# lzzcd001/MeshDiffusion

Measured on NVIDIA H100. Metric: denoising sample-steps/sec at res-64 (4x64^3), uncond_gen PC sampler, higher is better.
Workload: dtype bf16x3

## Files before the change

include/meshdiff_b200.h:

```cpp
#ifndef MESHDIFF_B200_H
#define MESHDIFF_B200_H

#ifdef __cplusplus
extern "C" {
#endif

const char* mdb_last_error(void);
int mdb_version(void);

typedef struct mdb_unet mdb_unet;

typedef struct mdb_unet_config {
  int image_size;
  int nf;
  int n_levels;
  int ch_mult[8];
  int num_res_blocks;
  int level0_blocks;
  int n_attn;
  int attn_resolutions[4];
  int num_channels;
  int stem_ksize;
  int use_pos_bias;
  int max_batch;
  int precision;
  int training;
} mdb_unet_config;

int mdb_unet_create(const mdb_unet_config* cfg, mdb_unet** out);
int mdb_unet_create_dry(const mdb_unet_config* cfg, mdb_unet** out);
void mdb_unet_destroy(mdb_unet* net);

int mdb_unet_num_params(mdb_unet* net);
int mdb_unet_param_info(mdb_unet* net, int idx, const char** name, long long* numel, int* ndim, long long* shape8);
int mdb_unet_set_param(mdb_unet* net, const char* name, const float* src, long long numel, int src_is_device,
                       void* stream);
int mdb_unet_set_params(mdb_unet* net, int count, const char* const* names, const float* const* srcs, const long long* numels,
                        void* stream);
int mdb_unet_get_param(mdb_unet* net, const char* name, float* dst, long long numel, int dst_is_device, void* stream);
int mdb_unet_commit(mdb_unet* net, void* stream);
int mdb_unet_forward(mdb_unet* net, const float* x, const float* labels, float* out, int batch, void* stream);
int mdb_unet_info(mdb_unet* net, double* flops_per_sample, long long* arena_bytes, int* n_gemm_launches, int* n_steps);
int mdb_unet_gemm_ops(mdb_unet* net, int i, const char** name, double* flops, double* fill_bytes);
int mdb_unet_gemm_slots(mdb_unet* net, int i, int* a_slots, int* b_slots, int* smem_bytes);
int mdb_unet_gemm_tiles(mdb_unet* net, int i, int* work_items, int* splits, int* ksteps, int* entry_ksteps, int* block_n);
int mdb_unet_profile(mdb_unet* net, const float* x, const float* labels, float* out, int batch, void* stream,
                     char* names_buf, int names_len, float* ms, int max_steps, int* n_steps);

int mdb_unet_set_dropout(mdb_unet* net, float p, unsigned long long seed);
int mdb_unet_backward(mdb_unet* net, const float* dout, float* grads, long long grads_numel, int batch, int accumulate,
                      void* stream);
int mdb_unet_grad_offset(mdb_unet* net, const char* name, long long* offset);
int mdb_unet_backward_input(mdb_unet* net, const float* dout, float* dx, float* grads, long long grads_numel, int batch,
                            int accumulate, void* stream);
int mdb_unet_grad_ready(mdb_unet* net, const char* name, int* n_launches);
int mdb_unet_backward_marked(mdb_unet* net, const float* dout, float* grads, long long grads_numel, int batch,
                             int accumulate, const int* mark_steps, void* const* mark_events, int n_marks, void* stream);
int mdb_unet_debug_stats(mdb_unet* net, long long* host_out, long long capacity, long long* count);
int mdb_unet_train_info(mdb_unet* net, double* bwd_flops_per_sample, int* n_bwd_steps, long long* total_param_numel);
int mdb_unet_profile_backward(mdb_unet* net, const float* dout, float* grads, int batch, void* stream, char* names_buf,
                              int names_len, float* ms, int max_steps, int* n_steps);

int mdb_fingerprint(const void* const* ptrs_dev, const long long* numels_dev, int n, unsigned long long* out_dev,
                    void* stream);

typedef struct mdb_sampler_cond {
  const float* partial;
  long long partial_bstride;
  const float* partial_mask;
  long long mask_bstride;
  int channel;
  float mean_coef, std;
  const float* noise;
} mdb_sampler_cond;

int mdb_sampler_update(const float* eps, float* x, float* x_mean, const float* noise, const float* mask, float beta,
                       float std, long long voxels, int channels, int batch, unsigned long long seed,
                       unsigned long long offset, const mdb_sampler_cond* cond , void* stream);
int mdb_sampler_run(mdb_unet* net, float* x, float* x_mean, const float* mask, const float* labels,
                    const float* betas, const float* stds, int n_steps, int batch, unsigned long long seed,
                    float* eps_buf, float* labels_buf, int step0, const mdb_sampler_cond* cond ,
                    const float* cond_mean_coefs, const float* cond_stds, int cond_until, void* stream);

typedef struct mdb_solver_step {
  float label;
  float sigma, inv_alpha;
  float c_x, c_0, c_1, c_z;
  float cond_coef, cond_std;
} mdb_solver_step;

int mdb_solver_update(const float* eps, float* x, float* x0_hist, const float* mask, const mdb_solver_step* step,
                      long long voxels, int channels, int batch, const float* noise ,
                      unsigned long long seed, unsigned long long offset, const mdb_sampler_cond* cond ,
                      void* stream);
int mdb_solver_run(mdb_unet* net, float* x, float* x0_hist, const float* mask, const mdb_solver_step* steps, int n_steps,
                   int batch, unsigned long long seed, float* eps_buf, float* labels_buf, int step0,
                   const mdb_sampler_cond* cond , int cond_until, void* stream);

int mdb_ddpm_loss(const float* pred, const float* noise, const float* mask, double mask_sum, float* loss_out,
                  float* grad_pred, double* scratch, int batch, int channels, long long voxels, void* stream);
int mdb_ddpm_perturb(const float* x0, const float* noise, const float* mask, const float* sqrt_ac,
                     const float* sqrt_1mac, float* out, int batch, int channels, long long voxels, void* stream);
int mdb_chunk_elems(void);
int mdb_grad_clip_coef(const float* const* grads_dev, const long long* numels_dev, const int* chunks_dev, int n_chunks,
                       float max_norm, float* coef_out, float* total_norm_out, double* scratch, void* stream);
int mdb_adam_ema_step(float* const* params_dev, const float* const* grads_dev, float* const* exp_avg_dev,
                      float* const* exp_avg_sq_dev, float* const* ema_dev, const long long* numels_dev,
                      const int* chunks_dev, int n_chunks, float lr, float beta1, float beta2, float eps,
                      float weight_decay, int step, const float* clip_coef_dev, float ema_decay, void* stream);
int mdb_ema_update(float* const* ema_dev, const float* const* params_dev, const long long* numels_dev,
                   const int* chunks_dev, int n_chunks, float ema_decay, void* stream);

int mdb_allreduce_grads(void* nccl_comm, float* grads, long long numel, int world_size, void* stream);

int mdb_conv3d(const void* x, int batch, int cin, int z, int y_, int x_, const float* w, const float* bias, int cout,
               int ksize, int stride, void* out, const float* rowbias, const void* residual, long long* stats,
               int precision, void* stream);
int mdb_groupnorm_act(const void* x, const long long* stats, const float* gamma, const float* beta, void* y, int batch,
                      long long voxels, int channels, int silu, int precision, void* stream);

int mdb_conv3d_backward(const void* dy, const void* x, const float* w, int batch, int cin, int cout, int z, int y_,
                        int x_, int ksize, int stride, float* dw, void* dx, void* stream);
int mdb_conv3d_backward_prec(const void* dy, const void* x, const float* w, int batch, int cin, int cout, int z, int y_,
                             int x_, int ksize, int stride, float* dw, void* dx, int precision, void* stream);
int mdb_groupnorm_act_backward(const void* x, const long long* stats, const float* gamma, const float* beta,
                               void* da, const void* add, void* dx, float* dgamma, float* dbeta, int batch,
                               long long voxels, int channels, int silu, float dropout_p, unsigned long long seed,
                               void* stream);
int mdb_groupnorm_act_backward_prec(const void* x, const long long* stats, const float* gamma, const float* beta,
                                    void* da, const void* add, void* dx, float* dgamma, float* dbeta, int batch,
                                    long long voxels, int channels, int silu, float dropout_p, unsigned long long seed,
                                    int precision, void* stream);

int mdb_marching_tets_prepare(const int* tets_host, int n_tets, int n_verts, int max_batch, void** handle);
void mdb_marching_tets_destroy(void* handle);
int mdb_marching_tets_info(void* handle, int* n_edges, int* uv_grid_n);
int mdb_marching_tets_uvs(void* handle, float* uvs, void* stream);
int mdb_marching_tets_count(void* handle, const float* sdf, int batch, int* counts_host, void* stream);
int mdb_marching_tets_extract(void* handle, const float* pos, long long pos_batch_stride, const float* sdf, int batch,
                              float* verts, long long* faces, long long* uv_idx, long long* face_to_tet,
                              long long* valid_vert_idx, const long long* vert_off, const long long* face_off,
                              const long long* vv_off, void* stream);
int mdb_marching_tets_vertex_ids(void* handle, int batch, unsigned* out, void* stream);
int mdb_marching_tets_backward(void* handle, const float* pos, long long pos_batch_stride, const float* sdf, int batch,
                               const unsigned* vertex_ids, const float* grad_verts, const long long* vert_off,
                               float* grad_pos, float* grad_sdf, void* stream);

int mdb_mesh_auto_normals(const float* v_pos, const long long* faces, int n_verts, int n_faces, float* v_nrm, float* f_nrm,
                          long long* scratch, void* stream);
int mdb_mesh_compute_tangents(const float* v_pos, const long long* t_pos_idx, const float* v_tex, const long long* t_tex_idx,
                              const float* v_nrm, const long long* t_nrm_idx, int n_nrm, int n_faces, float* v_tng,
                              long long* scratch, void* stream);

int mdb_mesh_sample_points(const float* verts, const long long* faces, const long long* vert_off, const long long* face_off,
                           int n_meshes, int n_points, const float* uniforms, unsigned long long seed, long long first_id,
                           double* cdf, float* points, int* n_written, void* stream);
int mdb_chamfer_matrix(const float* A, int nA, int N, const float* B, int nB, int M, double* out, void* stream);
int mdb_emd_matrix(const float* A, int nA, const float* B, int nB, int N, float eps, double* out, double* gap, void* stream);

int mdb_pflow_drift_div(const float* x, const float* e, const float* h, const float* g, const float* mask, float beta, float std,
                        float* drift, double* div, int batch, int channels, long long voxels, void* stream);

int mdb_raster_depth(const float* verts, const long long* faces, const long long* vert_off, const long long* face_off,
                     const int* job_mesh, const float* mvp, int n_jobs, int res, unsigned long long* scratch, float* depth,
                     int* face_id, int* n_behind, void* stream);
int mdb_visible_tets(const float* pos, long long pos_stride, const int* tets, int n_tets, const long long* face_to_tet,
                     const long long* face_off, const int* job_mesh, const float* mvp, int n_jobs, int res, const float* depth,
                     const int* face_id, unsigned char* visible, unsigned char* rast, void* stream);

#ifdef __cplusplus
}
#endif
#endif
```

meshdiffusion_b200/_native.py:

```python
import ctypes
import os

_HERE = os.path.dirname(os.path.abspath(__file__))
LIB_PATH = os.path.join(_HERE, "lib", "libmeshdiff_b200.so")

_lib = None


class NativeError(RuntimeError):
    pass


class UNetConfigC(ctypes.Structure):
    _fields_ = [
        ("image_size", ctypes.c_int),
        ("nf", ctypes.c_int),
        ("n_levels", ctypes.c_int),
        ("ch_mult", ctypes.c_int * 8),
        ("num_res_blocks", ctypes.c_int),
        ("level0_blocks", ctypes.c_int),
        ("n_attn", ctypes.c_int),
        ("attn_resolutions", ctypes.c_int * 4),
        ("num_channels", ctypes.c_int),
        ("stem_ksize", ctypes.c_int),
        ("use_pos_bias", ctypes.c_int),
        ("max_batch", ctypes.c_int),
        ("precision", ctypes.c_int),
        ("training", ctypes.c_int),
    ]


class SamplerCondC(ctypes.Structure):
    _fields_ = [
        ("partial", ctypes.c_void_p), ("partial_bstride", ctypes.c_longlong),
        ("partial_mask", ctypes.c_void_p), ("mask_bstride", ctypes.c_longlong),
        ("channel", ctypes.c_int), ("mean_coef", ctypes.c_float), ("std", ctypes.c_float),
        ("noise", ctypes.c_void_p),
    ]


class SolverStepC(ctypes.Structure):
    _fields_ = [(name, ctypes.c_float) for name in
                ("label", "sigma", "inv_alpha", "c_x", "c_0", "c_1", "c_z", "cond_coef", "cond_std")]


_vp, _i, _ll, _f, _u64, _d = ctypes.c_void_p, ctypes.c_int, ctypes.c_longlong, ctypes.c_float, ctypes.c_ulonglong, ctypes.c_double
SIGNATURES = {
    "mdb_last_error": (ctypes.c_char_p, []),
    "mdb_version": (_i, []),
    "mdb_unet_create": (_i, [ctypes.POINTER(UNetConfigC), ctypes.POINTER(_vp)]),
    "mdb_unet_create_dry": (_i, [ctypes.POINTER(UNetConfigC), ctypes.POINTER(_vp)]),
    "mdb_unet_destroy": (None, [_vp]),
    "mdb_unet_num_params": (_i, [_vp]),
    "mdb_unet_param_info": (_i, [_vp, _i, ctypes.POINTER(ctypes.c_char_p), ctypes.POINTER(_ll), ctypes.POINTER(_i), ctypes.POINTER(_ll)]),
    "mdb_unet_set_param": (_i, [_vp, ctypes.c_char_p, _vp, _ll, _i, _vp]),
    "mdb_unet_get_param": (_i, [_vp, ctypes.c_char_p, _vp, _ll, _i, _vp]),
    "mdb_unet_commit": (_i, [_vp, _vp]),
    "mdb_unet_set_params": (_i, [_vp, _i, _vp, _vp, _vp, _vp]),
    "mdb_unet_forward": (_i, [_vp, _vp, _vp, _vp, _i, _vp]),
    "mdb_unet_info": (_i, [_vp, ctypes.POINTER(_d), ctypes.POINTER(_ll), ctypes.POINTER(_i), ctypes.POINTER(_i)]),
    "mdb_unet_gemm_ops": (_i, [_vp, _i, ctypes.POINTER(ctypes.c_char_p), ctypes.POINTER(_d), ctypes.POINTER(_d)]),
    "mdb_unet_gemm_slots": (_i, [_vp, _i, ctypes.POINTER(_i), ctypes.POINTER(_i), ctypes.POINTER(_i)]),
    "mdb_unet_gemm_tiles": (_i, [_vp, _i, ctypes.POINTER(_i), ctypes.POINTER(_i), ctypes.POINTER(_i), ctypes.POINTER(_i),
                                 ctypes.POINTER(_i)]),
    "mdb_unet_profile": (_i, [_vp, _vp, _vp, _vp, _i, _vp, ctypes.c_char_p, _i, ctypes.POINTER(_f), _i, ctypes.POINTER(_i)]),
    "mdb_unet_set_dropout": (_i, [_vp, _f, _u64]),
    "mdb_unet_backward": (_i, [_vp, _vp, _vp, _ll, _i, _i, _vp]),
    "mdb_unet_grad_offset": (_i, [_vp, ctypes.c_char_p, ctypes.POINTER(_ll)]),
    "mdb_unet_backward_input": (_i, [_vp, _vp, _vp, _vp, _ll, _i, _i, _vp]),
    "mdb_unet_grad_ready": (_i, [_vp, ctypes.c_char_p, ctypes.POINTER(_i)]),
    "mdb_unet_backward_marked": (_i, [_vp, _vp, _vp, _ll, _i, _i, ctypes.POINTER(_i), ctypes.POINTER(_vp), _i, _vp]),
    "mdb_unet_debug_stats": (_i, [_vp, _vp, _ll, ctypes.POINTER(_ll)]),
    "mdb_unet_train_info": (_i, [_vp, ctypes.POINTER(_d), ctypes.POINTER(_i), ctypes.POINTER(_ll)]),
    "mdb_unet_profile_backward": (_i, [_vp, _vp, _vp, _i, _vp, ctypes.c_char_p, _i, ctypes.POINTER(_f), _i, ctypes.POINTER(_i)]),
    "mdb_fingerprint": (_i, [_vp, _vp, _i, _vp, _vp]),
    "mdb_sampler_update": (_i, [_vp, _vp, _vp, _vp, _vp, _f, _f, _ll, _i, _i, _u64, _u64, ctypes.POINTER(SamplerCondC), _vp]),
    "mdb_sampler_run": (_i, [_vp, _vp, _vp, _vp, ctypes.POINTER(_f), ctypes.POINTER(_f), ctypes.POINTER(_f), _i, _i, _u64, _vp, _vp,
                             _i, ctypes.POINTER(SamplerCondC), ctypes.POINTER(_f), ctypes.POINTER(_f), _i, _vp]),
    "mdb_solver_update": (_i, [_vp, _vp, _vp, _vp, ctypes.POINTER(SolverStepC), _ll, _i, _i, _vp, _u64, _u64,
                               ctypes.POINTER(SamplerCondC), _vp]),
    "mdb_solver_run": (_i, [_vp, _vp, _vp, _vp, ctypes.POINTER(SolverStepC), _i, _i, _u64, _vp, _vp, _i,
                            ctypes.POINTER(SamplerCondC), _i, _vp]),
    "mdb_ddpm_loss": (_i, [_vp, _vp, _vp, _d, _vp, _vp, _vp, _i, _i, _ll, _vp]),
    "mdb_ddpm_perturb": (_i, [_vp, _vp, _vp, _vp, _vp, _vp, _i, _i, _ll, _vp]),
    "mdb_chunk_elems": (_i, []),
    "mdb_grad_clip_coef": (_i, [_vp, _vp, _vp, _i, _f, _vp, _vp, _vp, _vp]),
    "mdb_adam_ema_step": (_i, [_vp, _vp, _vp, _vp, _vp, _vp, _vp, _i, _f, _f, _f, _f, _f, _i, _vp, _f, _vp]),
    "mdb_ema_update": (_i, [_vp, _vp, _vp, _vp, _i, _f, _vp]),
    "mdb_allreduce_grads": (_i, [_vp, _vp, _ll, _i, _vp]),
    "mdb_conv3d": (_i, [_vp, _i, _i, _i, _i, _i, _vp, _vp, _i, _i, _i, _vp, _vp, _vp, _vp, _i, _vp]),
    "mdb_groupnorm_act": (_i, [_vp, _vp, _vp, _vp, _vp, _i, _ll, _i, _i, _i, _vp]),
    "mdb_conv3d_backward": (_i, [_vp, _vp, _vp, _i, _i, _i, _i, _i, _i, _i, _i, _vp, _vp, _vp]),
    "mdb_groupnorm_act_backward": (_i, [_vp, _vp, _vp, _vp, _vp, _vp, _vp, _vp, _vp, _i, _ll, _i, _i, _f, _u64, _vp]),
    "mdb_conv3d_backward_prec": (_i, [_vp, _vp, _vp, _i, _i, _i, _i, _i, _i, _i, _i, _vp, _vp, _i, _vp]),
    "mdb_groupnorm_act_backward_prec": (_i, [_vp, _vp, _vp, _vp, _vp, _vp, _vp, _vp, _vp, _i, _ll, _i, _i, _f, _u64, _i, _vp]),
    "mdb_marching_tets_prepare": (_i, [_vp, _i, _i, _i, ctypes.POINTER(_vp)]),
    "mdb_marching_tets_destroy": (None, [_vp]),
    "mdb_marching_tets_info": (_i, [_vp, ctypes.POINTER(_i), ctypes.POINTER(_i)]),
    "mdb_marching_tets_uvs": (_i, [_vp, _vp, _vp]),
    "mdb_marching_tets_count": (_i, [_vp, _vp, _i, ctypes.POINTER(_i), _vp]),
    "mdb_mesh_auto_normals": (_i, [_vp, _vp, _i, _i, _vp, _vp, _vp, _vp]),
    "mdb_mesh_compute_tangents": (_i, [_vp, _vp, _vp, _vp, _vp, _vp, _i, _i, _vp, _vp, _vp]),
    "mdb_marching_tets_extract": (_i, [_vp, _vp, _ll, _vp, _i, _vp, _vp, _vp, _vp, _vp, _vp, _vp, _vp, _vp]),
    "mdb_marching_tets_vertex_ids": (_i, [_vp, _i, _vp, _vp]),
    "mdb_marching_tets_backward": (_i, [_vp, _vp, _ll, _vp, _i, _vp, _vp, _vp, _vp, _vp, _vp]),
    "mdb_mesh_sample_points": (_i, [_vp, _vp, _vp, _vp, _i, _i, _vp, _u64, _ll, _vp, _vp, _vp, _vp]),
    "mdb_chamfer_matrix": (_i, [_vp, _i, _i, _vp, _i, _i, _vp, _vp]),
    "mdb_emd_matrix": (_i, [_vp, _i, _vp, _i, _i, _f, _vp, _vp, _vp]),
    "mdb_pflow_drift_div": (_i, [_vp, _vp, _vp, _vp, _vp, _f, _f, _vp, _vp, _i, _i, _ll, _vp]),
    "mdb_raster_depth": (_i, [_vp, _vp, _vp, _vp, _vp, _vp, _i, _i, _vp, _vp, _vp, _vp, _vp]),
    "mdb_visible_tets": (_i, [_vp, _ll, _vp, _i, _vp, _vp, _vp, _vp, _i, _i, _vp, _vp, _vp, _vp, _vp]),
}


def lib():
    global _lib
    if _lib is not None:
        return _lib
    if not os.path.exists(LIB_PATH):
        from . import build as _build
        _build.build()
    if not os.path.exists(LIB_PATH):
        raise NativeError("libmeshdiff_b200.so is missing and could not be built; there is no fallback path")
    L = ctypes.CDLL(LIB_PATH)
    for name, (res, args) in SIGNATURES.items():
        fn = getattr(L, name)
        fn.restype = res
        fn.argtypes = args
    _lib = L
    return L


def check(code):
    if code != 0:
        raise NativeError(lib().mdb_last_error().decode())


def ptr(t):
    if t is None:
        return None
    return ctypes.c_void_p(t.data_ptr())


def current_stream():
    import torch
    return ctypes.c_void_p(torch.cuda.current_stream().cuda_stream)
```

meshdiffusion_b200/csrc/api.cu:

```cuda
#include "../../include/meshdiff_b200.h"
#include "unet.h"
#include <cstring>
#include <cmath>

using namespace mdb;

static thread_local std::string g_err;
namespace mdb { void set_last_error(const std::string& msg) { g_err = msg; } }

#define MDB_API_BEGIN try {
#define MDB_API_END                         \
  }                                         \
  catch (const std::exception& e) {         \
    g_err = e.what();                       \
    return 1;                               \
  }                                         \
  catch (...) {                             \
    g_err = "mdb: unknown error";           \
    return 2;                               \
  }                                         \
  return 0;

struct mdb_unet { UNet* net; };

extern "C" {

const char* mdb_last_error(void) { return g_err.c_str(); }
int mdb_version(void) { return 100; }

static int create_impl(const mdb_unet_config* c, mdb_unet** out, bool dry) {
  MDB_API_BEGIN
  if (!c || !out) throw std::runtime_error("mdb: null argument");
  UNetConfig u;
  u.image_size = c->image_size; u.nf = c->nf; u.n_levels = c->n_levels;
  for (int i = 0; i < 8; ++i) u.ch_mult[i] = c->ch_mult[i];
  u.num_res_blocks = c->num_res_blocks; u.level0_blocks = c->level0_blocks;
  u.n_attn = c->n_attn;
  for (int i = 0; i < 4; ++i) u.attn_resolutions[i] = c->attn_resolutions[i];
  u.num_channels = c->num_channels; u.stem_ksize = c->stem_ksize; u.use_pos_bias = c->use_pos_bias;
  u.max_batch = c->max_batch; u.precision = c->precision; u.training = c->training;
  auto* h = new mdb_unet;
  h->net = nullptr;
  try { h->net = new UNet(u, dry); } catch (...) { delete h; throw; }
  *out = h;
  MDB_API_END
}

int mdb_unet_create(const mdb_unet_config* c, mdb_unet** out) { return create_impl(c, out, false); }
int mdb_unet_create_dry(const mdb_unet_config* c, mdb_unet** out) { return create_impl(c, out, true); }

void mdb_unet_destroy(mdb_unet* n) {
  if (!n) return;
  delete n->net;
  delete n;
}

int mdb_unet_num_params(mdb_unet* n) { return n ? (int)n->net->params().size() : -1; }

int mdb_unet_param_info(mdb_unet* n, int idx, const char** name, long long* numel, int* ndim, long long* shape8) {
  MDB_API_BEGIN
  const auto& ps = n->net->params();
  if (idx < 0 || idx >= (int)ps.size()) throw std::runtime_error("mdb: parameter index out of range");
  if (name) *name = ps[idx].name.c_str();
  if (numel) *numel = ps[idx].numel;
  if (ndim) *ndim = (int)ps[idx].shape.size();
  if (shape8) for (size_t i = 0; i < ps[idx].shape.size() && i < 8; ++i) shape8[i] = ps[idx].shape[i];
  MDB_API_END
}

int mdb_unet_set_param(mdb_unet* n, const char* name, const float* src, long long numel, int dev, void* stream) {
  MDB_API_BEGIN
  n->net->set_param(name, src, numel, dev != 0, (cudaStream_t)stream);
  MDB_API_END
}

int mdb_unet_set_params(mdb_unet* n, int count, const char* const* names, const float* const* srcs, const long long* numels,
                        void* stream) {
  MDB_API_BEGIN
  for (int i = 0; i < count; ++i) n->net->set_param(names[i], srcs[i], numels[i], true, (cudaStream_t)stream);
  MDB_API_END
}

int mdb_unet_get_param(mdb_unet* n, const char* name, float* dst, long long numel, int dev, void* stream) {
  MDB_API_BEGIN
  n->net->get_param(name, dst, numel, dev != 0, (cudaStream_t)stream);
  MDB_API_END
}

int mdb_unet_commit(mdb_unet* n, void* stream) {
  MDB_API_BEGIN
  n->net->commit((cudaStream_t)stream);
  MDB_API_END
}

int mdb_unet_forward(mdb_unet* n, const float* x, const float* labels, float* out, int B, void* stream) {
  MDB_API_BEGIN
  n->net->forward(x, labels, out, B, (cudaStream_t)stream);
  MDB_API_END
}

int mdb_unet_info(mdb_unet* n, double* flops, long long* arena, int* ngemm, int* nsteps) {
  MDB_API_BEGIN
  if (flops) *flops = n->net->flops_per_sample();
  if (arena) *arena = (long long)n->net->arena_bytes();
  if (ngemm) *ngemm = n->net->num_gemm_launches();
  if (nsteps) *nsteps = n->net->num_steps();
  MDB_API_END
}

int mdb_unet_gemm_ops(mdb_unet* n, int i, const char** name, double* flops, double* fill_bytes) {
  MDB_API_BEGIN
  if (i < 0 || i >= n->net->num_gemm_launches()) throw std::runtime_error("mdb: GEMM launch index out of range");
  const GemmOp& g = n->net->gemm(i);
  if (name) *name = g.name.c_str();
  if (flops) *flops = g.flops;
  if (fill_bytes) *fill_bytes = g.fill_bytes();
  MDB_API_END
}

int mdb_unet_gemm_slots(mdb_unet* n, int i, int* a_slots, int* b_slots, int* smem_bytes) {
  MDB_API_BEGIN
  if (i < 0 || i >= n->net->num_gemm_launches()) throw std::runtime_error("mdb: GEMM launch index out of range");
  int a = 0, b = 0, sm = 0;
  n->net->gemm(i).slots(a, b, sm);
  if (a_slots) *a_slots = a;
  if (b_slots) *b_slots = b;
  if (smem_bytes) *smem_bytes = sm;
  MDB_API_END
}

int mdb_unet_gemm_tiles(mdb_unet* n, int i, int* work_items, int* splits, int* ksteps, int* entry_ksteps, int* block_n) {
  MDB_API_BEGIN
  if (i < 0 || i >= n->net->num_gemm_launches()) throw std::runtime_error("mdb: GEMM launch index out of range");
  const GemmOp& g = n->net->gemm(i);
  const int s = g.p.splits > 1 ? g.p.splits : 1;
  int nk = 0;
  for (const LoadEntry& e : g.loads) nk = e.nk > nk ? e.nk : nk;
  if (work_items) *work_items = g.p.tx * g.p.ty * g.p.tz * g.p.tb * g.p.n_tiles_n * s;
  if (splits) *splits = s;
  if (ksteps) *ksteps = g.ksteps;
  if (entry_ksteps) *entry_ksteps = nk;
  if (block_n) *block_n = g.block_n;
  MDB_API_END
}

int mdb_unet_profile(mdb_unet* n, const float* x, const float* labels, float* out, int B, void* stream, char* names,
                     int names_len, float* ms, int max_steps, int* nsteps) {
  MDB_API_BEGIN
  auto r = n->net->profile(x, labels, out, B, (cudaStream_t)stream);
  std::string all;
  int k = 0;
  for (auto& p : r) {
    if (k >= max_steps) break;
    all += p.first; all += "\n";
    ms[k++] = p.second;
  }
  if ((int)all.size() + 1 > names_len) throw std::runtime_error("mdb: names buffer too small");
  std::memcpy(names, all.c_str(), all.size() + 1);
  if (nsteps) *nsteps = k;
  MDB_API_END
}

int mdb_unet_set_dropout(mdb_unet* n, float p, unsigned long long seed) {
  MDB_API_BEGIN
  n->net->set_dropout(p, seed);
  MDB_API_END
}

int mdb_unet_backward(mdb_unet* n, const float* dout, float* grads, long long grads_numel, int B, int accumulate, void* stream) {
  MDB_API_BEGIN
  if (grads_numel != n->net->total_param_numel()) throw std::runtime_error("mdb: gradient buffer has the wrong size");
  n->net->backward(dout, grads, B, accumulate != 0, (cudaStream_t)stream);
  MDB_API_END
}

int mdb_unet_backward_marked(mdb_unet* n, const float* dout, float* grads, long long grads_numel, int B, int accumulate,
                             const int* mark_steps, void* const* mark_events, int n_marks, void* stream) {
  MDB_API_BEGIN
  if (grads_numel != n->net->total_param_numel()) throw std::runtime_error("mdb: gradient buffer has the wrong size");
  if (n_marks > 0 && (!mark_steps || !mark_events)) throw std::runtime_error("mdb: null mark arrays");
  n->net->backward(dout, grads, B, accumulate != 0, (cudaStream_t)stream, mark_steps, mark_events, n_marks);
  MDB_API_END
}

int mdb_unet_backward_input(mdb_unet* n, const float* dout, float* dx, float* grads, long long grads_numel, int B, int accumulate,
                            void* stream) {
  MDB_API_BEGIN
  if (grads && grads_numel != n->net->total_param_numel()) throw std::runtime_error("mdb: gradient buffer has the wrong size");
  n->net->backward_input(dout, dx, grads, B, accumulate != 0, (cudaStream_t)stream);
  MDB_API_END
}

int mdb_unet_grad_ready(mdb_unet* n, const char* name, int* step) {
  MDB_API_BEGIN
  *step = n->net->grad_ready_step(name);
  MDB_API_END
}

int mdb_unet_grad_offset(mdb_unet* n, const char* name, long long* off) {
  MDB_API_BEGIN
  *off = n->net->grad_offset(name);
  MDB_API_END
}

int mdb_unet_debug_stats(mdb_unet* n, long long* host_out, long long capacity, long long* count) {
  MDB_API_BEGIN
  const long long c = (long long)n->net->stats_count();
  if (count) *count = c;
  if (host_out) {
    if (capacity < c) throw std::runtime_error("mdb: stats buffer too small");
    MDB_CUDA_CHECK(cudaMemcpy(host_out, n->net->stats_ptr(), (size_t)c * sizeof(long long), cudaMemcpyDeviceToHost));
  }
  MDB_API_END
}

int mdb_unet_train_info(mdb_unet* n, double* bwd_flops, int* nsteps, long long* numel) {
  MDB_API_BEGIN
  if (bwd_flops) *bwd_flops = n->net->bwd_flops_per_sample();
  if (nsteps) *nsteps = n->net->num_bwd_steps();
  if (numel) *numel = n->net->total_param_numel();
  MDB_API_END
}

int mdb_unet_profile_backward(mdb_unet* n, const float* dout, float* grads, int B, void* stream, char* names, int names_len,
                              float* ms, int max_steps, int* nsteps) {
  MDB_API_BEGIN
  auto r = n->net->profile_backward(dout, grads, B, (cudaStream_t)stream);
  std::string all;
  int k = 0;
  for (auto& p : r) {
    if (k >= max_steps) break;
    all += p.first; all += "\n";
    ms[k++] = p.second;
  }
  if ((int)all.size() + 1 > names_len) throw std::runtime_error("mdb: names buffer too small");
  std::memcpy(names, all.c_str(), all.size() + 1);
  if (nsteps) *nsteps = k;
  MDB_API_END
}

static void set_cond(SamplerUpdateArgs& a, const mdb_sampler_cond* c, float coef, float stdv) {
  if (!c || !c->partial) return;
  if (!c->partial_mask) throw std::runtime_error("mdb: conditional sampling needs partial_mask");
  if (c->channel < 0 || c->channel >= a.C) throw std::runtime_error("mdb: partial_channel out of range");
  a.cond_partial = c->partial; a.cond_partial_bs = c->partial_bstride;
  a.cond_pmask = c->partial_mask; a.cond_pmask_bs = c->mask_bstride;
  a.cond_channel = c->channel; a.cond_coef = coef; a.cond_std = stdv; a.cond_noise = c->noise;
}

int mdb_sampler_update(const float* eps, float* x, float* x_mean, const float* noise, const float* mask, float beta,
                       float stdv, long long V, int C, int B, unsigned long long seed, unsigned long long offset,
                       const mdb_sampler_cond* cond, void* stream) {
  MDB_API_BEGIN
  SamplerUpdateArgs a{};
  a.eps = eps; a.x = x; a.x_mean = x_mean; a.noise = noise; a.mask = mask; a.beta = beta; a.stdv = stdv;
  a.V = V; a.C = C; a.seed = seed; a.offset = offset;
  if (cond) set_cond(a, cond, cond->mean_coef, cond->std);
  launch_sampler_update(a, B, (cudaStream_t)stream);
  MDB_API_END
}

__global__ void fingerprint_kernel(const unsigned int* const* ptrs, const long long* numels, unsigned long long* out) {
  const int t = blockIdx.y;
  const unsigned int* p = ptrs[t];
  const long long n = numels[t];
  unsigned long long h = 0;
  for (long long i = blockIdx.x * (long long)blockDim.x + threadIdx.x; i < n; i += (long long)gridDim.x * blockDim.x)
    h += (unsigned long long)p[i] * (0x9E3779B97F4A7C15ull * (unsigned long long)(i + 1) | 1ull);
  for (int o = 16; o; o >>= 1) h += __shfl_xor_sync(0xffffffffu, h, o);
  if ((threadIdx.x & 31) == 0 && h) atomicAdd(out + t, h);
}

int mdb_fingerprint(const void* const* ptrs_dev, const long long* numels_dev, int n, unsigned long long* out_dev, void* stream) {
  MDB_API_BEGIN
  cudaStream_t s = (cudaStream_t)stream;
  MDB_CUDA_CHECK(cudaMemsetAsync(out_dev, 0, (size_t)n * 8, s));
  fingerprint_kernel<<<dim3(64, n), 256, 0, s>>>(reinterpret_cast<const unsigned int* const*>(ptrs_dev), numels_dev, out_dev);
  MDB_CUDA_CHECK(cudaGetLastError());
  MDB_API_END
}

__global__ void fill_kernel(float* p, float v, int n) {
  const int i = blockIdx.x * blockDim.x + threadIdx.x;
  if (i < n) p[i] = v;
}

int mdb_sampler_run(mdb_unet* n, float* x, float* x_mean, const float* mask, const float* labels, const float* betas,
                    const float* stds, int n_steps, int B, unsigned long long seed, float* eps_buf, float* labels_buf,
                    int step0, const mdb_sampler_cond* cond, const float* cond_mean_coefs, const float* cond_stds,
                    int cond_until, void* stream) {
  MDB_API_BEGIN
  cudaStream_t s = (cudaStream_t)stream;
  const UNetConfig& c = n->net->cfg();
  const long long V = (long long)c.image_size * c.image_size * c.image_size;
  if (cond && cond->partial && (!cond_mean_coefs || !cond_stds)) throw std::runtime_error("mdb: conditional run needs the marginal_prob tables");
  if (cond && cond->noise) throw std::runtime_error("mdb: mdb_sampler_run draws its noise in-kernel (cond->noise must be NULL)");
  for (int i = 0; i < n_steps; ++i) {
    fill_kernel<<<(B + 127) / 128, 128, 0, s>>>(labels_buf, labels[i], B);
    n->net->forward(x, labels_buf, eps_buf, B, s, true);
    SamplerUpdateArgs a{};
    a.eps = eps_buf; a.x = x; a.x_mean = x_mean; a.noise = nullptr; a.mask = mask; a.beta = betas[i]; a.stdv = stds[i];
    a.V = V; a.C = c.num_channels; a.seed = seed; a.offset = 4ull * (unsigned long long)(step0 + i);
    if (cond && step0 + i < cond_until) set_cond(a, cond, cond_mean_coefs[i], cond_stds[i]);
    launch_sampler_update(a, B, s);
  }
  MDB_API_END
}

static SolverUpdateArgs solver_args(const float* eps, float* x, float* x0_hist, const float* mask, const mdb_solver_step& st,
                                    long long V, int C, const mdb_sampler_cond* c) {
  SolverUpdateArgs a{};
  a.eps = eps; a.x = x; a.x0_hist = x0_hist; a.mask = mask;
  a.sigma = st.sigma; a.inv_alpha = st.inv_alpha; a.c_x = st.c_x; a.c_0 = st.c_0; a.c_1 = st.c_1; a.c_z = st.c_z;
  a.V = V; a.C = C;
  if (c && c->partial) {
    if (!c->partial_mask) throw std::runtime_error("mdb: conditional sampling needs partial_mask");
    if (c->channel < 0 || c->channel >= C) throw std::runtime_error("mdb: partial_channel out of range");
    a.cond_partial = c->partial; a.cond_partial_bs = c->partial_bstride;
    a.cond_pmask = c->partial_mask; a.cond_pmask_bs = c->mask_bstride;
    a.cond_channel = c->channel; a.cond_coef = st.cond_coef; a.cond_std = st.cond_std; a.cond_noise = c->noise;
  }
  return a;
}

int mdb_solver_update(const float* eps, float* x, float* x0_hist, const float* mask, const mdb_solver_step* step,
                      long long V, int C, int B, const float* noise, unsigned long long seed, unsigned long long offset,
                      const mdb_sampler_cond* cond, void* stream) {
  MDB_API_BEGIN
  if (!step) throw std::runtime_error("mdb: mdb_solver_update needs a step");
  if (V <= 0 || C <= 0 || B <= 0) throw std::runtime_error("mdb: mdb_solver_update needs positive voxels, channels, batch");
  SolverUpdateArgs a = solver_args(eps, x, x0_hist, mask, *step, V, C, cond);
  a.noise = noise; a.seed = seed; a.offset = offset;
  launch_solver_update(a, B, (cudaStream_t)stream);
  MDB_API_END
}

int mdb_solver_run(mdb_unet* n, float* x, float* x0_hist, const float* mask, const mdb_solver_step* steps, int n_steps,
                   int B, unsigned long long seed, float* eps_buf, float* labels_buf, int step0,
                   const mdb_sampler_cond* cond, int cond_until, void* stream) {
  MDB_API_BEGIN
  cudaStream_t s = (cudaStream_t)stream;
  const UNetConfig& c = n->net->cfg();
  const long long V = (long long)c.image_size * c.image_size * c.image_size;
  if (n_steps > 0 && !steps) throw std::runtime_error("mdb: mdb_solver_run needs the step table");
  if (cond && cond->noise) throw std::runtime_error("mdb: mdb_solver_run draws its noise in-kernel (cond->noise must be NULL)");
  for (int i = 0; i < n_steps; ++i) {
    fill_kernel<<<(B + 127) / 128, 128, 0, s>>>(labels_buf, steps[i].label, B);
    n->net->forward(x, labels_buf, eps_buf, B, s, true);
    SolverUpdateArgs a = solver_args(eps_buf, x, x0_hist, mask, steps[i], V, c.num_channels,
                                     step0 + i < cond_until ? cond : nullptr);
    a.noise = nullptr; a.seed = seed; a.offset = 4ull * (unsigned long long)(step0 + i);
    launch_solver_update(a, B, s);
  }
  MDB_API_END
}

int mdb_conv3d(const void* x, int B, int cin, int z, int y_, int x_, const float* w, const float* bias, int cout,
               int ksize, int stride, void* out, const float* rowbias, const void* residual, long long* stats,
               int precision, void* stream) {
  MDB_API_BEGIN
  cudaStream_t s = (cudaStream_t)stream;
  const Precision pr = precision_from_int(precision);
  const int xo = x_ / stride, yo = y_ / stride, zo = z / stride;
  GemmOp g;
  g.set_output(pr, xo, yo, zo, B, cout, out, cout, false);
  Act a; a.ptr = const_cast<void*>(x); a.C = cin; a.X = x_; a.Y = y_; a.Z = z; a.B = B;
  if (ksize == 1) g.add_pointwise({a}, w, false);
  else g.add_conv({a}, w, ksize, stride);
  if (bias) g.set_bias(bias);
  if (rowbias) g.set_rowbias(rowbias, cout);
  if (residual) g.set_residual(residual, cout, (long long)xo * yo * zo * cout, false);
  if (stats) g.set_stats(stats);
  g.finalize();
  g.upload(s);
  g.repack(s);
  g.launch(s);
  MDB_CUDA_CHECK(cudaStreamSynchronize(s));
  MDB_API_END
}

int mdb_groupnorm_act(const void* x, const long long* stats, const float* gamma, const float* beta, void* y, int B,
                      long long V, int C, int silu, int precision, void* stream) {
  MDB_API_BEGIN
  if (!stats) throw std::runtime_error("mdb: GroupNorm needs the per-channel statistics of x (stats)");
  cudaStream_t s = (cudaStream_t)stream;
  NormActArgs na{};
  na.x0 = x; na.C0 = C; na.ld0 = C; na.x1 = nullptr; na.C1 = 0; na.ld1 = 0;
  na.y = y; na.voxels = V; na.silu = silu; na.prec = precision_from_int(precision);
  na.stats0 = stats; na.stats1 = nullptr; na.gamma = gamma; na.beta = beta; na.groups = 32; na.eps = 1e-6f;
  launch_norm_act(na, B, s);
  MDB_CUDA_CHECK(cudaStreamSynchronize(s));
  MDB_API_END
}

int mdb_conv3d_backward(const void* dy, const void* x, const float* w, int B, int cin, int cout, int z, int y_, int x_,
                        int ksize, int stride, float* dw, void* dx, void* stream) {
  return mdb_conv3d_backward_prec(dy, x, w, B, cin, cout, z, y_, x_, ksize, stride, dw, dx, 0, stream);
}

int mdb_conv3d_backward_prec(const void* dy, const void* x, const float* w, int B, int cin, int cout, int z, int y_, int x_,
                             int ksize, int stride, float* dw, void* dx, int precision, void* stream) {
  MDB_API_BEGIN
  cudaStream_t s = (cudaStream_t)stream;
  const Precision pr = precision_from_int(precision);
  if (pr == kTF32) throw std::runtime_error("mdb: conv3d backward takes bf16 (0) or bf16x3 (2) operands");
  const int xo = x_ / stride, yo = y_ / stride, zo = z / stride;
  Act ady; ady.ptr = const_cast<void*>(dy); ady.C = cout; ady.X = xo; ady.Y = yo; ady.Z = zo; ady.B = B;
  Act ax; ax.ptr = const_cast<void*>(x); ax.C = cin; ax.X = x_; ax.Y = y_; ax.Z = z; ax.B = B;
  if (dw) {
    const int T = ksize * ksize * ksize;
    const WgradPlan pl = plan_wgrad(xo, yo, zo, B, cout, cin, ksize, stride, pr);
    float* scratch = nullptr;
    MDB_CUDA_CHECK(cudaMalloc(&scratch, pl.scratch_bytes));
    WgradOut o; o.ptr = dw; o.sm = (long long)cin * T; o.sn = T; o.st = 1;
    WgradOp op;
    op.init(ady, ax, ksize, stride, o, scratch, pr);
    op.launch(s, B, false);
    MDB_CUDA_CHECK(cudaStreamSynchronize(s));
    cudaFree(scratch);
  }
  if (dx) {
    if (stride != 1) throw std::runtime_error("mdb: conv3d data gradient entry point supports stride 1");
    GemmOp g;
    g.set_output(pr, x_, y_, z, B, cin, dx, cin, false);
    if (ksize == 1) { WSrc ws{w, 1, (long long)cin, 0, cout}; g.add_pointwise_w({ady}, &ws); }
    else g.add_conv_dgrad(ady, w, cin, ksize);
    g.finalize();
    g.upload(s);
    g.repack(s);
    g.launch(s);
    MDB_CUDA_CHECK(cudaStreamSynchronize(s));
  }
  MDB_API_END
}

int mdb_groupnorm_act_backward(const void* x, const long long* stats, const float* gamma, const float* beta, void* da,
                               const void* add, void* dx, float* dgamma, float* dbeta, int B, long long V, int C, int silu,
                               float dropout_p, unsigned long long seed, void* stream) {
  return mdb_groupnorm_act_backward_prec(x, stats, gamma, beta, da, add, dx, dgamma, dbeta, B, V, C, silu, dropout_p, seed, 0, stream);
}

int mdb_groupnorm_act_backward_prec(const void* x, const long long* stats, const float* gamma, const float* beta, void* da,
                                    const void* add, void* dx, float* dgamma, float* dbeta, int B, long long V, int C, int silu,
                                    float dropout_p, unsigned long long seed, int precision, void* stream) {
  MDB_API_BEGIN
  if (!stats) throw std::runtime_error("mdb: GroupNorm backward needs the forward statistics of x (stats)");
  cudaStream_t s = (cudaStream_t)stream;
  const Precision pr = precision_from_int(precision);
  if (pr == kTF32) throw std::runtime_error("mdb: GroupNorm backward takes bf16 (0) or bf16x3 (2) operands");
  float *part = nullptr, *sums = nullptr;
  MDB_CUDA_CHECK(cudaMalloc(&part, (size_t)kBwdPartRows(B) * C * 2 * sizeof(float)));
  MDB_CUDA_CHECK(cudaMalloc(&sums, (size_t)B * C * 2 * sizeof(float)));
  GnBwdArgs a{};
  a.x0 = x; a.C0 = C; a.ld0 = C; a.stats0 = stats; a.gamma = gamma; a.beta = beta; a.da = da;
  a.voxels = V; a.silu = silu; a.groups = 32; a.eps = 1e-6f;
  const DropoutParams d = dropout_params(dropout_p);
  a.drop_thresh = d.thresh; a.drop_scale = d.scale; a.seed = seed;
  a.part = part; a.sums = sums; a.dgamma = dgamma; a.dbeta = dbeta; a.accumulate = 0;
  a.dx = dx; a.add0 = add; a.add0_ld = C;
  a.prec = pr;
  launch_gn_bwd_reduce(a, B, s);
  launch_gn_bwd_apply(a, B, s);
  MDB_CUDA_CHECK(cudaStreamSynchronize(s));
  cudaFree(part); cudaFree(sums);
  MDB_API_END
}

}
```

meshdiffusion_b200/csrc/gemm_host.cu:

```cuda
#include "gemm_host.h"
#include "elementwise.cuh"
#include <cstring>
#include <cstdlib>
#include <mutex>

namespace mdb {

typedef CUresult (*PFN_encodeTiled)(CUtensorMap*, CUtensorMapDataType, cuuint32_t, void*, const cuuint64_t*,
                                    const cuuint64_t*, const cuuint32_t*, const cuuint32_t*, CUtensorMapInterleave,
                                    CUtensorMapSwizzle, CUtensorMapL2promotion, CUtensorMapFloatOOBfill);

static PFN_encodeTiled get_encode() {
  static PFN_encodeTiled fn = nullptr;
  static std::once_flag once;
  std::call_once(once, [] {
    void* f = nullptr;
    cudaDriverEntryPointQueryResult q;
    cudaError_t e = cudaGetDriverEntryPoint("cuTensorMapEncodeTiled", &f, cudaEnableDefault, &q);
    if (e != cudaSuccess || q != cudaDriverEntryPointSuccess || !f)
      throw std::runtime_error("mdb: cuTensorMapEncodeTiled not available (needs an sm_90+ driver)");
    fn = reinterpret_cast<PFN_encodeTiled>(f);
  });
  return fn;
}

void encode_map(CUtensorMap* m, Precision prec, const MapDesc& d) {
  cuuint64_t gd[5], gs[4];
  cuuint32_t bd[5], es[5];
  for (int i = 0; i < d.rank; ++i) { gd[i] = d.dims[i]; bd[i] = d.box[i]; es[i] = 1; }
  for (int i = 0; i + 1 < d.rank; ++i) gs[i] = d.strides[i];
  CUtensorMapDataType dt = prec == kTF32 ? CU_TENSOR_MAP_DATA_TYPE_FLOAT32 : CU_TENSOR_MAP_DATA_TYPE_BFLOAT16;
  CUresult r = get_encode()(m, dt, d.rank, d.base, gd, gs, bd, es, CU_TENSOR_MAP_INTERLEAVE_NONE,
                            CU_TENSOR_MAP_SWIZZLE_128B, CU_TENSOR_MAP_L2_PROMOTION_L2_256B,
                            CU_TENSOR_MAP_FLOAT_OOB_FILL_NONE);
  if (r != CUDA_SUCCESS) {
    std::string msg = "mdb: cuTensorMapEncodeTiled failed (" + std::to_string((int)r) + ") rank " +
                      std::to_string(d.rank) + " dims";
    for (int i = 0; i < d.rank; ++i) msg += " " + std::to_string(d.dims[i]);
    msg += " box";
    for (int i = 0; i < d.rank; ++i) msg += " " + std::to_string(d.box[i]);
    throw std::runtime_error(msg);
  }
}

template <int BN, Precision P, bool GNB>
static void launch_impl(const GemmParams& p, int grid, int smem, cudaStream_t stream) {
  static bool configured[64] = {};
  auto kern = gemm_tc_kernel<BN, P, GNB>;
  int dev = 0;
  MDB_CUDA_CHECK(cudaGetDevice(&dev));
  if (dev >= 64 || !configured[dev]) {
    MDB_CUDA_CHECK(cudaFuncSetAttribute(kern, cudaFuncAttributeMaxDynamicSharedMemorySize, kMaxDynSmem));
    if (dev < 64) configured[dev] = true;
  }
  kern<<<grid, kGemmThreads, smem, stream>>>(p);
  MDB_CUDA_CHECK(cudaGetLastError());
}

struct GemmVariant {
  void (*launch)(const GemmParams&, int grid, int smem, cudaStream_t);
  int fixed_bytes;
};
template <int BN, Precision P, bool GNB>
static GemmVariant variant() { return {launch_impl<BN, P, GNB>, GemmCfg<BN, GNB>::kFixedBytes}; }
template <int BN>
static GemmVariant variant(Precision prec, bool gnb) {
  if (gnb) {
    if (prec == kTF32) throw std::runtime_error("mdb: the GroupNorm-backward epilogue is built for bf16 / split-bf16 operands");
    return prec == kBF16X3 ? variant<BN, kBF16X3, true>() : variant<BN, kBF16, true>();
  }
  return prec == kTF32 ? variant<BN, kTF32, false>() : prec == kBF16X3 ? variant<BN, kBF16X3, false>() : variant<BN, kBF16, false>();
}
static GemmVariant gemm_variant(int block_n, Precision prec, bool gnb) {
  return block_n == 32 ? variant<32>(prec, gnb) : variant<128>(prec, gnb);
}

int GemmOp::pick_slots(GemmParams& q) const {
  const int fixed = gemm_variant(block_n, prec, gnb).fixed_bytes;
  const int budget = kMaxDynSmem - fixed;
  q.a_slot_bytes = (a_slot_need + 1023) / 1024 * 1024;
  q.b_slot_bytes = parts(prec) * block_n * kRowBytes;
  auto env_cap = [](const char* name, int def) {
    int cap = def;
    if (const char* e = getenv(name)) { const int c = atoi(e); if (c >= 2) cap = c; }
    return cap < kMaxSlots ? cap : kMaxSlots;
  };
  const int cap = env_cap("MDB_MAX_STAGES", 4), bcap = env_cap("MDB_MAX_BSLOTS", kMaxSlots);
  int na = 2, nb = 2;
  int used = na * q.a_slot_bytes + nb * q.b_slot_bytes;
  if (used > budget) throw std::runtime_error("mdb: operand rings need at least two slots each");
  for (;;) {
    if (nb < na * nk_max && nb < bcap && used + q.b_slot_bytes <= budget) { ++nb; used += q.b_slot_bytes; }
    else if (na < cap && used + q.a_slot_bytes <= budget) { ++na; used += q.a_slot_bytes; }
    else break;
  }
  q.n_aslots = na;
  q.n_bslots = nb;
  return fixed + used;
}

void GemmOp::slots(int& a_slots, int& b_slots, int& smem_bytes) const {
  GemmParams q = p;
  smem_bytes = pick_slots(q);
  a_slots = q.n_aslots;
  b_slots = q.n_bslots;
}

double GemmOp::fill_bytes(int B) const {
  double per_tile = 0;
  for (const auto& e : loads) per_tile += parts(prec) * ((double)e.rows * kRowBytes + (double)e.nk * block_n * kRowBytes);
  const int tb = B > 0 ? (B + p.bb - 1) / p.bb : p.tb;
  return per_tile * p.tx * p.ty * p.tz * tb * p.n_tiles_n;
}

int sm_count() {
  static int n = 0;
  if (!n) {
    int dev = 0;
    MDB_CUDA_CHECK(cudaGetDevice(&dev));
    MDB_CUDA_CHECK(cudaDeviceGetAttribute(&n, cudaDevAttrMultiProcessorCount, dev));
  }
  return n;
}

Geometry pick_geometry(int X, int Y, int Z) {
  if (Y == 1 && Z == 1) return {128, 1, 1, 1};
  int bx = X < 8 ? X : 8;
  int by = 128 / bx;
  if (by > 16) by = 16;
  if (by > Y) by = Y;
  int rem = 128 / (bx * by);
  int bz = rem < Z ? rem : Z;
  int bb = rem / bz;
  return {bx, by, bz, bb};
}

int plan_splits(int X, int Y, int Z, int B, int N, int cin_total, int taps, Precision prec) {
  const Geometry g = pick_geometry(X, Y, Z);
  const int tiles_m = ((X + g.bx - 1) / g.bx) * ((Y + g.by - 1) / g.by) * ((Z + g.bz - 1) / g.bz) * ((B + g.bb - 1) / g.bb);
  const int block_n = N <= 32 ? 32 : 128;
  const int tiles = tiles_m * ((N + block_n - 1) / block_n);
  const int kprod = ((cin_total + kb_elems(prec) - 1) / kb_elems(prec)) * taps * (prec == kBF16X3 ? 3 : 1);
  if (tiles > 49 || kprod < 48) return 1;
  int S = kPlanSMs / tiles;
  if (S > 16) S = 16;
  if (S > kprod / 8) S = kprod / 8;
  return S < 2 ? 1 : S;
}

void GemmOp::enable_splits(int S, float* scratch) {
  if (S <= 1) return;
  if (p.ocs != 1 || p.out_fp32 || p.bias_on_m || p.alpha != 1.f || p.res_fp32)
    throw std::runtime_error("mdb: split-K is only wired for plain NDHWC conv outputs");
  if (p.osx != (long long)p.N * parts(prec) || (p.rsx && p.rsx != (long long)p.N * parts(prec)))
    throw std::runtime_error("mdb: split-K needs dense [B][V][N] output / residual");
  splits = S;
  p.splits = S;
  p.partial = scratch;
  p.split_stride = (long long)p.Bn * p.X * p.Y * p.Z * p.N;
}

GemmOp::~GemmOp() {
  if (d_loads) cudaFree(d_loads);
  if (d_ks0) cudaFree(d_ks0);
  if (d_wpacked && owns_w) cudaFree(d_wpacked);
}

static long long physical_strides(bool split, long long lo_off, long long& sx, long long& sy, long long& sz, long long& sb) {
  if (!split) return 0;
  sx *= 2; sy *= 2; sz *= 2; sb *= 2;
  return lo_off;
}

void GemmOp::set_output_strided(Precision pr, int X, int Y, int Z, int B, int N, void* out, long long osx,
                                long long osy, long long osz, long long osb, bool out_fp32, long long lo_off) {
  prec = pr;
  geo = pick_geometry(X, Y, Z);
  if (geo.bx * geo.by * geo.bz * geo.bb != kBlockM) throw std::runtime_error("mdb: unsupported tile geometry");
  if (geo.bb > 1 && (geo.bx * geo.by * geo.bz) % 32 != 0)
    throw std::runtime_error("mdb: multi-sample tiles need a multiple of 32 rows per sample");
  if (geo.bb > 4) throw std::runtime_error("mdb: at most 4 samples per tile");
  p.bx = geo.bx; p.by = geo.by; p.bz = geo.bz; p.bb = geo.bb;
  p.X = X; p.Y = Y; p.Z = Z; p.Bn = B;
  p.tx = (X + geo.bx - 1) / geo.bx; p.ty = (Y + geo.by - 1) / geo.by;
  p.tz = (Z + geo.bz - 1) / geo.bz; p.tb = (B + geo.bb - 1) / geo.bb;
  p.N = N;
  block_n = N <= 32 ? 32 : 128;
  p.n_tiles_n = (N + block_n - 1) / block_n;
  p.out = out;
  p.osx = osx; p.osy = osy; p.osz = osz; p.osb = osb;
  p.out_fp32 = out_fp32 ? 1 : 0;
  p.out_lo_off = physical_strides(prec == kBF16X3 && !out_fp32, lo_off >= 0 ? lo_off : osx, p.osx, p.osy, p.osz, p.osb);
  p.alpha = 1.f;
  p.ocs = 1;
  p.kb_elems = kb_elems(prec);
}

void GemmOp::set_output(Precision pr, int X, int Y, int Z, int B, int N, void* out, long long ldc, bool out_fp32) {
  set_output_strided(pr, X, Y, Z, B, N, out, ldc, ldc * X, ldc * X * Y, ldc * X * Y * Z, out_fp32);
}

MapDesc act_map(const Act& a, Precision prec, int part, Geometry box, int sub, int px, int py, int pz) {
  const long long es = esize(prec);
  const long long sx = a.row() * parts(prec) * es, sy = sx * a.X, sz = sy * a.Y, sb = sz * a.Z;
  MapDesc m;
  m.rank = 5;
  m.base = static_cast<char*>(a.ptr) + (long long)part * a.row() * es + px * sx + py * sy + pz * sz;
  m.dims[0] = a.C; m.dims[1] = (a.X - px + sub - 1) / sub; m.dims[2] = (a.Y - py + sub - 1) / sub;
  m.dims[3] = (a.Z - pz + sub - 1) / sub; m.dims[4] = a.B;
  m.strides[0] = sx * sub; m.strides[1] = sy * sub; m.strides[2] = sz * sub; m.strides[3] = sb;
  m.box[0] = kb_elems(prec); m.box[1] = box.bx; m.box[2] = box.by; m.box[3] = box.bz; m.box[4] = box.bb;
  return m;
}

int GemmOp::add_amap(const Act& a, int halo, int sub, int px, int py, int pz, int part) {
  if ((int)amaps_.size() >= kMaxAMaps) throw std::runtime_error("mdb: too many A tensor maps");
  if (halo > 0 && (geo.bz != 1 || geo.bb != 1)) throw std::runtime_error("mdb: halo needs a (bx,by,1,1) tile");
  amaps_.push_back(act_map(a, prec, part, {geo.bx, geo.by + halo, geo.bz, geo.bb}, sub, px, py, pz));
  return (int)amaps_.size() - 1;
}

void GemmOp::add_load_x(int tm_hi, int tm_lo, int nk, int rows, int jrows, int dx, int dy, int dz, int c0, int wsrc,
                        int wc0, int tap0, int tapj) {
  if ((int)loads.size() >= kMaxLoads) throw std::runtime_error("mdb: load table overflow");
  if (rows > kAStageRows) throw std::runtime_error("mdb: A box exceeds the stage size");
  LoadEntry e{};
  e.tmap = (uint8_t)tm_hi; e.tmap_lo = (uint8_t)(prec == kBF16X3 ? tm_lo : tm_hi);
  e.nk = (uint8_t)nk; e.rows = (uint8_t)rows; e.jrows = (uint8_t)jrows;
  e.dx = (int8_t)dx; e.dy = (int8_t)dy; e.dz = (int8_t)dz; e.wsrc = (uint8_t)wsrc;
  e.c0 = (uint16_t)c0; e.wc0 = (uint16_t)wc0; e.tap0 = (uint8_t)tap0; e.tapj = (uint8_t)tapj;
  loads.push_back(e);
  ksteps += nk;
}

void GemmOp::add_conv(const std::vector<Act>& srcs, const float* w, int k, int stride) {
  int ctot = 0;
  for (auto& s : srcs) ctot += s.C;
  const int T = k * k * k;
  add_conv_w(srcs, WSrc{w, 1LL * ctot * T, (long long)T, 1, ctot}, k, stride);
}

void GemmOp::add_conv_dgrad(const Act& dy, const float* w_oidhw, int cin_total, int k) {
  const int T = k * k * k;
  add_conv_w({dy}, WSrc{w_oidhw + (T - 1), (long long)T, 1LL * cin_total * T, -1, dy.C}, k, 1);
}

void GemmOp::add_conv_w(const std::vector<Act>& srcs, const WSrc& wsrc, int k, int stride) {
  const int KB = kb_elems(prec);
  int ctot = 0;
  for (auto& s : srcs) ctot += s.C;
  const int T = k * k * k;
  const int ws = add_wsrc(wsrc);
  const int pad = k / 2;
  flops += 2.0 * p.X * p.Y * p.Z * p.Bn * (double)p.N * ctot * T;
  int coff = 0;
  if (stride == 1) {
    const bool reuse = geo.bz == 1 && geo.bb == 1 && geo.bx * (geo.by + k - 1) <= kAStageRows && p.Y >= geo.by;
    const bool x3 = prec == kBF16X3;
    for (auto& s : srcs) {
      const int tm = add_amap(s, reuse ? k - 1 : 0);
      const int tl = x3 ? add_amap(s, reuse ? k - 1 : 0, 1, 0, 0, 0, 1) : tm;
      for (int c0 = 0; c0 < s.C; c0 += KB) {
        if (reuse) {
          for (int dz = 0; dz < k; ++dz)
            for (int dx = 0; dx < k; ++dx)
              add_load_x(tm, tl, k, geo.bx * (geo.by + k - 1), geo.bx, dx - pad, -pad, dz - pad, c0, ws, coff + c0,
                         (dz * k) * k + dx, k);
        } else {
          for (int dz = 0; dz < k; ++dz)
            for (int dy = 0; dy < k; ++dy)
              for (int dx = 0; dx < k; ++dx)
                add_load_x(tm, tl, 1, kBlockM, 0, dx - pad, dy - pad, dz - pad, c0, ws, coff + c0, (dz * k + dy) * k + dx, 0);
        }
      }
      coff += s.C;
    }
  } else if (stride == 2) {
    if (k != 3) throw std::runtime_error("mdb: stride-2 conv supports k=3 only");
    const bool x3 = prec == kBF16X3;
    for (auto& s : srcs) {
      int tm[8], tl[8];
      for (int par = 0; par < 8; ++par) tm[par] = add_amap(s, 0, 2, par & 1, (par >> 1) & 1, (par >> 2) & 1);
      for (int par = 0; par < 8; ++par) tl[par] = x3 ? add_amap(s, 0, 2, par & 1, (par >> 1) & 1, (par >> 2) & 1, 1) : tm[par];
      for (int c0 = 0; c0 < s.C; c0 += KB)
        for (int dz = 0; dz < 3; ++dz)
          for (int dy = 0; dy < 3; ++dy)
            for (int dx = 0; dx < 3; ++dx) {
              const int par = (dx & 1) | ((dy & 1) << 1) | ((dz & 1) << 2);
              add_load_x(tm[par], tl[par], 1, kBlockM, 0, dx >> 1, dy >> 1, dz >> 1, c0, ws, coff + c0, (dz * 3 + dy) * 3 + dx, 0);
            }
      coff += s.C;
    }
  } else {
    throw std::runtime_error("mdb: unsupported stride");
  }
}

void GemmOp::add_conv_up2(const Act& s, const float* w8, int px, int py, int pz) {
  const int KB = kb_elems(prec);
  const int ws = add_wsrc(WSrc{w8, 8LL * s.C, 8, 1, s.C});
  flops += 2.0 * p.X * p.Y * p.Z * p.Bn * (double)p.N * s.C * 8;
  const bool x3 = prec == kBF16X3;
  const bool reuse = geo.bz == 1 && geo.bb == 1 && geo.bx * (geo.by + 1) <= kAStageRows && p.Y >= geo.by;
  const int tm = add_amap(s, reuse ? 1 : 0);
  const int tl = x3 ? add_amap(s, reuse ? 1 : 0, 1, 0, 0, 0, 1) : tm;
  for (int c0 = 0; c0 < s.C; c0 += KB) {
    for (int ez = 0; ez < 2; ++ez)
      for (int ex = 0; ex < 2; ++ex) {
        if (reuse) {
          add_load_x(tm, tl, 2, geo.bx * (geo.by + 1), geo.bx, ex - 1 + px, -1 + py, ez - 1 + pz, c0, ws, c0, (ez * 2) * 2 + ex, 2);
        } else {
          for (int ey = 0; ey < 2; ++ey)
            add_load_x(tm, tl, 1, kBlockM, 0, ex - 1 + px, ey - 1 + py, ez - 1 + pz, c0, ws, c0, (ez * 2 + ey) * 2 + ex, 0);
        }
      }
  }
}

void GemmOp::add_pointwise(const std::vector<Act>& srcs, const float* w, bool w_in_out) {
  int ctot = 0;
  for (auto& s : srcs) ctot += s.C;
  WSrc ws = w_in_out ? WSrc{w, 1, (long long)p.N, 0, ctot} : WSrc{w, (long long)ctot, 1, 0, ctot};
  add_pointwise_w(srcs, &ws);
}

void GemmOp::add_pointwise_w(const std::vector<Act>& srcs, const WSrc* w) {
  const int KB = kb_elems(prec);
  int ctot = 0;
  for (auto& s : srcs) ctot += s.C;
  int ws = 0;
  if (w) ws = add_wsrc(*w);
  flops += 2.0 * p.X * p.Y * p.Z * p.Bn * (double)p.N * ctot;
  int coff = 0;
  for (auto& s : srcs) {
    const int tm = add_amap(s, 0);
    const int tl = prec == kBF16X3 ? add_amap(s, 0, 1, 0, 0, 0, 1) : tm;
    for (int c0 = 0; c0 < s.C; c0 += KB) add_load_x(tm, tl, 1, kBlockM, 0, 0, 0, 0, c0, ws, coff + c0, 0, 0);
    coff += s.C;
  }
}

void GemmOp::set_residual(const void* res, long long ldr, long long batch_stride, bool fp32) {
  p.res = res;
  p.batch_fastest = batch_stride == 0 ? 1 : 0;
  p.rsx = ldr; p.rsy = ldr * p.X; p.rsz = ldr * p.X * p.Y; p.rsb = batch_stride;
  p.res_fp32 = fp32 ? 1 : 0;
  p.res_lo_off = physical_strides(prec == kBF16X3 && !fp32, ldr, p.rsx, p.rsy, p.rsz, p.rsb);
}

void GemmOp::set_gn_backward(const void* x0, long long ld0, int c0, const void* x1, long long ld1, const void* consts, int silu,
                             float* part) {
  if (prec == kTF32 || p.out_fp32 || p.ocs != 1)
    throw std::runtime_error("mdb: the GroupNorm-backward epilogue is built for bf16 / split-bf16 NDHWC outputs");
  if (p.N % 32 != 0 || (ld1 > 0 && c0 % 32 != 0)) throw std::runtime_error("mdb: GroupNorm-backward epilogue needs 32-channel aligned sources");
  if (splits > 1) throw std::runtime_error("mdb: GroupNorm-backward epilogue cannot be combined with split-K");
  gnb = true;
  p.res = x0; p.res_fp32 = 0; p.batch_fastest = 0;
  p.rsx = ld0; p.rsy = ld0 * p.X; p.rsz = ld0 * p.X * p.Y; p.rsb = ld0 * p.X * p.Y * p.Z;
  p.res1 = x1; p.res_c0 = ld1 > 0 ? c0 : p.N;
  p.r1sx = ld1; p.r1sy = ld1 * p.X; p.r1sz = ld1 * p.X * p.Y; p.r1sb = ld1 * p.X * p.Y * p.Z;
  p.res_lo_off = physical_strides(prec == kBF16X3, ld0, p.rsx, p.rsy, p.rsz, p.rsb);
  p.res1_lo_off = physical_strides(prec == kBF16X3, ld1, p.r1sx, p.r1sy, p.r1sz, p.r1sb);
  p.gnb_c = reinterpret_cast<const float4*>(consts);
  p.gnb_silu = silu;
  p.gnb_part = part;
}

MapDesc GemmOp::b_desc(void* ptr, long long K, int N, int batch, long long rsb, long long bsb) const {
  MapDesc m;
  m.base = ptr; m.rank = 3;
  m.dims[0] = (uint64_t)K; m.dims[1] = (uint64_t)N; m.dims[2] = (uint64_t)batch;
  m.strides[0] = (uint64_t)rsb; m.strides[1] = (uint64_t)bsb;
  m.box[0] = (uint32_t)kb_elems(prec); m.box[1] = (uint32_t)block_n; m.box[2] = 1;
  return m;
}

void GemmOp::set_b_activation(void* ptr, int K, int N, int batch, long long rs, long long bs) {
  b_from_act = true;
  p.b_batched = 1;
  const long long es = esize(prec);
  if (prec == kBF16X3) {
    if (K % kb_elems(prec) != 0) throw std::runtime_error("mdb: X3 activation-B operands need K to be a multiple of 64");
    b_lo_off = rs;
    bmap_ = b_desc(ptr, (int)(rs + K), N, batch, 2 * rs * es, 2 * bs * es);
    return;
  }
  bmap_ = b_desc(ptr, K, N, batch, rs * es, bs * es);
}

struct PackWSrc { const float* ptr; long long sn, sc, st; int cvalid; int ndiv; long long sn_hi; int cdiv; long long sc_hi; };
struct PackArgs { PackWSrc w[4]; };

template <Precision P>
__global__ void __launch_bounds__(256) pack_weights_kernel(const LoadEntry* __restrict__ loads, const int* __restrict__ load_ks0,
                                                         int n_loads, const __grid_constant__ PackArgs args, int N, int ksteps,
                                                         int KB, void* __restrict__ out) {
  const int vpk = KB >> 3;
  const long long total = 1LL * N * n_loads * vpk;
  for (long long idx = blockIdx.x * (long long)blockDim.x + threadIdx.x; idx < total; idx += (long long)gridDim.x * blockDim.x) {
    const int v8 = (int)(idx % vpk);
    const long long t = idx / vpk;
    const int l = (int)(t % n_loads);
    const int n = (int)(t / n_loads);
    const LoadEntry e = loads[l];
    const PackWSrc& w = args.w[e.wsrc];
    const long long noff = w.ndiv ? (long long)(n % w.ndiv) * w.sn + (long long)(n / w.ndiv) * w.sn_hi : (long long)n * w.sn;
    const int c0 = e.wc0 + v8 * 8;
    long long coff[8];
    unsigned valid = 0;
#pragma unroll
    for (int i = 0; i < 8; ++i) {
      const int c = c0 + i;
      if (c < w.cvalid) valid |= 1u << i;
      coff[i] = noff + (w.cdiv ? (long long)(c % w.cdiv) * w.sc + (long long)(c / w.cdiv) * w.sc_hi : (long long)c * w.sc);
    }
    const long long obase = ((long long)n * ksteps + load_ks0[l]) * parts(P) * KB + v8 * 8;
    for (int j = 0; j < e.nk; ++j) {
      const long long toff = (long long)(e.tap0 + j * e.tapj) * w.st;
      float v[8];
#pragma unroll
      for (int i = 0; i < 8; ++i) v[i] = (valid >> i) & 1u ? __ldg(w.ptr + coff[i] + toff) : 0.f;
      ActElem<P>* op = reinterpret_cast<ActElem<P>*>(out) + obase + (long long)j * parts(P) * KB;
      constexpr int E = kVecElems<P>;
#pragma unroll
      for (int i = 0; i < 8 / E; ++i) store_vec<P>(op + E * i, (long long)KB * sizeof(ActElem<P>), v + E * i);
    }
  }
}

void GemmOp::repack(cudaStream_t stream) {
  if (b_from_act) return;
  if (!d_ks0) {
    std::vector<int> ks0;
    int run = 0;
    for (size_t l = 0; l < loads.size(); ++l) { ks0.push_back(run); run += loads[l].nk; }
    if (run != ksteps) throw std::runtime_error("mdb: load table does not cover the packed K extent");
    MDB_CUDA_CHECK(cudaMalloc(&d_ks0, ks0.size() * sizeof(int)));
    MDB_CUDA_CHECK(cudaMemcpy(d_ks0, ks0.data(), ks0.size() * sizeof(int), cudaMemcpyHostToDevice));
  }
  if (wsrcs.size() > 4) throw std::runtime_error("mdb: too many weight sources");
  PackArgs args{};
  for (size_t i = 0; i < wsrcs.size(); ++i) args.w[i] = {wsrcs[i].ptr, wsrcs[i].sn, wsrcs[i].sc, wsrcs[i].st, wsrcs[i].cvalid, wsrcs[i].ndiv, wsrcs[i].sn_hi, wsrcs[i].cdiv, wsrcs[i].sc_hi};
  const int KB = kb_elems(prec), n_loads = (int)loads.size();
  const long long total = 1LL * p.N * n_loads * (KB / 8);
  int blocks = (int)((total + 255) / 256);
  if (blocks > kPlanSMs * 16) blocks = kPlanSMs * 16;
  if (prec == kTF32)
    pack_weights_kernel<kTF32><<<blocks, 256, 0, stream>>>(d_loads, d_ks0, n_loads, args, p.N, ksteps, KB, d_wpacked);
  else if (prec == kBF16X3)
    pack_weights_kernel<kBF16X3><<<blocks, 256, 0, stream>>>(d_loads, d_ks0, n_loads, args, p.N, ksteps, KB, d_wpacked);
  else
    pack_weights_kernel<kBF16><<<blocks, 256, 0, stream>>>(d_loads, d_ks0, n_loads, args, p.N, ksteps, KB, d_wpacked);
  MDB_CUDA_CHECK(cudaGetLastError());
}

void GemmOp::finalize() {
  if (loads.empty()) throw std::runtime_error("mdb: GemmOp without loads");
  p.b_explicit_k = 0;
  p.b_kstep = kb_elems(prec) * parts(prec);
  p.b_lo_k = kb_elems(prec);
  if (b_from_act) p.b_kstep = kb_elems(prec);
  if (b_from_act && prec == kBF16X3) {
    p.b_explicit_k = 1;
    p.b_lo_k = (int)b_lo_off;
  }
  if (!b_from_act) p.b_batched = 0;
  p.n_loads = (int)loads.size();
  if (p.splits < 1) p.splits = 1;
  {
    a_slot_need = 0;
    nk_max = 0;
    p.n_segs = 0;
    p.total_groups = 0;
    size_t i = 0;
    while (i < loads.size()) {
      size_t j = i;
      while (j < loads.size() && loads[j].nk == loads[i].nk && loads[j].rows == loads[i].rows && loads[j].jrows == loads[i].jrows) ++j;
      if (p.n_segs >= kMaxSegs) throw std::runtime_error("mdb: too many pipeline segments");
      GemmSeg sg{};
      sg.n_groups = (int)(j - i); sg.nk = loads[i].nk;
      sg.a_bytes = loads[i].rows * kRowBytes;
      sg.a_stride = (sg.a_bytes + 1023) / 1024 * 1024;
      sg.jbytes = loads[i].jrows * kRowBytes;
      const int need = parts(prec) * sg.a_stride;
      if (sg.a_stride > kAStageBytes) throw std::runtime_error("mdb: A box exceeds the slot size");
      if (need > a_slot_need) a_slot_need = need;
      if (sg.nk > nk_max) nk_max = sg.nk;
      p.segs[p.n_segs++] = sg;
      p.total_groups += sg.n_groups;
      i = j;
    }
  }
  if (p.splits > p.total_groups) { p.splits = p.total_groups; splits = p.splits; }
}

void GemmOp::upload(cudaStream_t stream) {
  for (size_t i = 0; i < amaps_.size(); ++i) encode_map(&p.amap[i], prec, amaps_[i]);
  MDB_CUDA_CHECK(cudaMalloc(&d_loads, loads.size() * sizeof(LoadEntry)));
  MDB_CUDA_CHECK(cudaMemcpyAsync(d_loads, loads.data(), loads.size() * sizeof(LoadEntry), cudaMemcpyHostToDevice, stream));
  p.loads = d_loads;
  if (!b_from_act) {
    const long long ktot = 1LL * ksteps * kb_elems(prec) * parts(prec);
    const long long bytes = ktot * p.N * esize(prec);
    MDB_CUDA_CHECK(cudaMalloc(&d_wpacked, bytes));
    owns_w = true;
    bmap_ = b_desc(d_wpacked, ktot, p.N, 1, ktot * esize(prec), bytes);
  }
  encode_map(&p.bmap, prec, bmap_);
  MDB_CUDA_CHECK(cudaStreamSynchronize(stream));
}

void GemmOp::launch(cudaStream_t stream, int B, void* out_override) const {
  GemmParams p = this->p;
  const int smem = pick_slots(p);
  if (B > 0) {
    if (B > this->p.Bn) throw std::runtime_error("mdb: batch exceeds the batch the op was built for");
    p.Bn = B;
    p.tb = (B + p.bb - 1) / p.bb;
  }
  if (out_override) p.out = out_override;
  const int tiles_m = p.tx * p.ty * p.tz * p.tb;
  const int total = tiles_m * p.n_tiles_n * (p.splits > 1 ? p.splits : 1);
  const int grid = total < sm_count() ? total : sm_count();
  if (gnb) {
    if (p.splits > 1) throw std::runtime_error("mdb: GroupNorm-backward epilogue: no split-K");
    p.gnb_drop_thresh = rt_drop_thresh; p.gnb_drop_scale = rt_drop_scale; p.gnb_seed = rt_seed;
  }
  gemm_variant(block_n, prec, gnb).launch(p, grid, smem, stream);
  if (p.splits > 1) {
    SplitReduceArgs a{};
    a.partial = p.partial; a.split_stride = p.split_stride; a.splits = p.splits;
    a.bias = p.bias; a.rowbias = p.rowbias; a.rowbias_ld = p.rowbias_ld;
    a.res = p.res; a.res_batch_stride = p.rsb;
    a.out = p.out; a.stats = p.stats; a.voxels = (long long)p.X * p.Y * p.Z; a.N = p.N; a.prec = prec;
    if (prec == kBF16X3) a.res_batch_stride = p.rsb / 2;
    launch_split_reduce(a, p.Bn, stream);
  }
}

}
```

meshdiffusion_b200/csrc/gemm_host.h:

```cpp
#pragma once
#include <cuda.h>
#include <cuda_runtime.h>
#include <stdint.h>
#include <string>
#include <vector>
#include <stdexcept>
#include "act_format.cuh"
#include "gemm_tc.cuh"

namespace mdb {

#define MDB_CUDA_CHECK(expr)                                                                         \
  do {                                                                                               \
    cudaError_t _e = (expr);                                                                         \
    if (_e != cudaSuccess)                                                                           \
      throw std::runtime_error(std::string("CUDA error ") + cudaGetErrorString(_e) + " at " + __FILE__ + ":" + \
                               std::to_string(__LINE__) + " (" #expr ")");                           \
  } while (0)

inline int kb_elems(Precision p) { return kRowBytes / esize(p); }

struct Act {
  void* ptr = nullptr;
  int C = 0, X = 0, Y = 0, Z = 0, B = 0;
  long long ld = 0;
  long long row() const { return ld ? ld : C; }
  long long voxels() const { return 1LL * X * Y * Z; }
  long long elems() const { return voxels() * B * C; }
};

struct WSrc {
  const float* ptr = nullptr;
  long long sn = 0, sc = 0, st = 0;
  int cvalid = 0;
  int ndiv = 0;
  long long sn_hi = 0;
  int cdiv = 0;
  long long sc_hi = 0;
};

struct Geometry { int bx, by, bz, bb; };
Geometry pick_geometry(int X, int Y, int Z);

struct MapDesc {
  void* base = nullptr;
  int rank = 0;
  uint64_t dims[5] = {}, strides[4] = {};
  uint32_t box[5] = {};
};
MapDesc act_map(const Act& a, Precision prec, int part, Geometry box, int sub = 1, int px = 0, int py = 0, int pz = 0);

class GemmOp {
 public:
  GemmParams p{};
  Precision prec = kBF16;
  int block_n = 128;
  int splits = 1;
  std::vector<LoadEntry> loads;
  std::vector<WSrc> wsrcs;
  int ksteps = 0;
  LoadEntry* d_loads = nullptr;
  int* d_ks0 = nullptr;
  void* d_wpacked = nullptr;
  bool owns_w = false;
  double flops = 0;
  std::string name;

  ~GemmOp();
  GemmOp() = default;
  GemmOp(const GemmOp&) = delete;
  GemmOp& operator=(const GemmOp&) = delete;

  void set_output(Precision prec, int X, int Y, int Z, int B, int N, void* out, long long ldc, bool out_fp32);
  void set_output_strided(Precision prec, int X, int Y, int Z, int B, int N, void* out, long long osx, long long osy,
                          long long osz, long long osb, bool out_fp32, long long lo_off = -1);
  int add_amap(const Act& a, int halo_rows_y, int sub_stride = 1, int px = 0, int py = 0, int pz = 0, int part = 0);
  void add_load_x(int tm_hi, int tm_lo, int nk, int rows, int jrows, int dx, int dy, int dz, int c0, int wsrc, int wc0,
                  int tap0, int tapj);
  int add_wsrc(const WSrc& w) { wsrcs.push_back(w); return (int)wsrcs.size() - 1; }

  void add_conv(const std::vector<Act>& srcs, const float* w_oidhw, int ksize, int stride);
  void add_conv_w(const std::vector<Act>& srcs, const WSrc& w, int ksize, int stride);
  void add_conv_up2(const Act& src, const float* w8, int px, int py, int pz);
  void add_conv_dgrad(const Act& dy, const float* w_oidhw, int cin_total, int ksize);
  void add_pointwise(const std::vector<Act>& srcs, const float* w, bool w_in_out);
  void add_pointwise_w(const std::vector<Act>& srcs, const WSrc* w);

  void set_b_activation(void* ptr, int K, int N, int batch, long long row_stride_elems, long long batch_stride_elems);

  void set_bias(const float* bias, bool on_m = false) { p.bias = bias; p.bias_on_m = on_m ? 1 : 0; }
  void set_rowbias(const float* rb, long long ld) { p.rowbias = rb; p.rowbias_ld = ld; }
  void set_out_col_stride(long long ocs) { p.ocs = ocs; }
  void set_residual(const void* res, long long ldr, long long batch_stride, bool fp32);
  void set_stats(long long* stats) { p.stats = stats; }
  void set_gn_backward(const void* x0, long long ld0, int c0, const void* x1, long long ld1, const void* consts, int silu, float* part);
  long long gnb_rows() const { return 1LL * p.tx * p.ty * p.tz * p.tb * p.bb; }
  int gnb_tiles_per_batch_tile() const { return p.tx * p.ty * p.tz; }
  int gnb_bb() const { return p.bb; }
  bool gnb = false;
  int rt_drop_thresh = 0; float rt_drop_scale = 1.f; unsigned long long rt_seed = 0;
  void set_alpha(float a) { p.alpha = a; }
  void enable_splits(int S, float* scratch);

  void finalize();
  void upload(cudaStream_t stream);
  void repack(cudaStream_t stream);
  void launch(cudaStream_t stream, int B = -1, void* out_override = nullptr) const;
  double fill_bytes(int B = -1) const;
  void slots(int& a_slots, int& b_slots, int& smem_bytes) const;

 private:
  Geometry geo{};
  bool b_from_act = false;
  int a_slot_need = 0;
  int nk_max = 0;
  int pick_slots(GemmParams& q) const;
  long long b_lo_off = 0;
  std::vector<MapDesc> amaps_;
  MapDesc bmap_;
  MapDesc b_desc(void* ptr, long long K, int N, int batch, long long row_stride_bytes, long long batch_stride_bytes) const;
};

int sm_count();
constexpr int kPlanSMs = 132;
void encode_map(CUtensorMap* m, Precision prec, const MapDesc& d);
int plan_splits(int X, int Y, int Z, int B, int N, int cin_total, int taps, Precision prec);

}
```

meshdiffusion_b200/csrc/gemm_tc.cuh:

```cuda
#pragma once
#include "ptx.cuh"
#include "act_format.cuh"
#include "gn_stats.cuh"

namespace mdb {

constexpr int kBlockM = 128;
constexpr int kRowBytes = 128;
constexpr int kAStageRows = 160;
constexpr int kAStageBytes = kAStageRows * kRowBytes;
constexpr int kMaxLoads = 2048;
constexpr int kMaxAMaps = 16;
constexpr int kGemmThreads = 384;
constexpr int kEpiThreads = 256;

struct __align__(16) LoadEntry {
  uint8_t tmap;
  uint8_t nk;
  uint8_t rows;
  uint8_t jrows;
  int8_t dx, dy, dz;
  uint8_t wsrc;
  uint16_t c0;
  uint16_t wc0;
  uint8_t tap0;
  uint8_t tapj;
  uint8_t tmap_lo;
  uint8_t pad;
};
static_assert(sizeof(LoadEntry) == 16, "LoadEntry must be 16 bytes");

struct GemmSeg {
  int n_groups;
  int nk;
  int a_bytes;
  int a_stride;
  int jbytes;
};
constexpr int kMaxSegs = 8;

struct GemmParams {
  CUtensorMap amap[kMaxAMaps];
  CUtensorMap bmap;
  const LoadEntry* loads;
  int n_loads;
  int n_segs;
  GemmSeg segs[kMaxSegs];
  int bx, by, bz, bb;
  int X, Y, Z, Bn;
  int tx, ty, tz, tb;
  int n_tiles_n;
  int N;
  int b_batched;
  int splits;
  int total_groups;
  float* partial;
  long long split_stride;
  int batch_fastest;
  int kb_elems;
  int b_explicit_k;
  int b_kstep;
  int b_lo_k;
  int n_aslots, a_slot_bytes, n_bslots, b_slot_bytes;
  long long out_lo_off, res_lo_off;
  void* out;
  long long osx, osy, osz, osb;
  long long ocs;
  int out_fp32;
  const float* bias;
  int bias_on_m;
  const float* rowbias;
  long long rowbias_ld;
  const void* res;
  long long rsx, rsy, rsz, rsb;
  int res_fp32;
  float alpha;
  long long* stats;
  const void* res1;
  long long r1sx, r1sy, r1sz, r1sb;
  long long res1_lo_off;
  int res_c0;
  const float4* gnb_c;
  int gnb_silu;
  int gnb_drop_thresh; float gnb_drop_scale; unsigned long long gnb_seed;
  float* gnb_part;
};

constexpr int kMaxSlots = 8;
constexpr int kMaxDynSmem = 232448;
template <int BLOCK_N, bool kWholeTile = false>
struct GemmCfg {
  static constexpr int kBTileBytes = BLOCK_N * kRowBytes;
  static constexpr int kStatsFloats = 24 * BLOCK_N;
  static constexpr int kStageCols = (kWholeTile || BLOCK_N < 64) ? BLOCK_N : 64;
  static constexpr int kStageRounds = BLOCK_N / kStageCols;
  static_assert(kStageRounds <= 2, "the epilogue stages at most two rounds");
  static constexpr int kAccPitch = kStageCols + 4;
  static constexpr int kAccFloats = kBlockM * kAccPitch;
  static constexpr int kFixedBytes = 1024 + kAccFloats * 4 + kStatsFloats * 4 + 4 * kMaxSlots * 8;
};
constexpr int kRegsProducer = 40, kRegsConsumer = 232;

__device__ __forceinline__ uint64_t kdesc(uint32_t saddr) { return make_wgmma_desc(saddr, 16, 1024); }

template <int OFF>
__device__ __forceinline__ void colsum_butterfly(float (&s)[32], float (&ss)[32], int lane) {
  const bool hi = (lane & OFF) != 0;
#pragma unroll
  for (int i = 0; i < OFF; ++i) {
    const float send_s = hi ? s[i] : s[i + OFF];
    const float send_q = hi ? ss[i] : ss[i + OFF];
    const float keep_s = hi ? s[i + OFF] : s[i];
    const float keep_q = hi ? ss[i + OFF] : ss[i];
    s[i] = keep_s + __shfl_xor_sync(0xffffffffu, send_s, OFF);
    ss[i] = keep_q + __shfl_xor_sync(0xffffffffu, send_q, OFF);
  }
  if constexpr (OFF > 1) colsum_butterfly<OFF / 2>(s, ss, lane);
}

template <Precision P>
__device__ __forceinline__ void add_res_chunk(const uint4 (&buf)[8], float (&v)[32]) {
  constexpr int E = kVecElems<P>, NV = 32 / E;
#pragma unroll
  for (int i = 0; i < NV; ++i) {
    float r[E];
    decode_vec<P>(buf[i], buf[P == kBF16X3 ? NV + i : i], r);
#pragma unroll
    for (int j = 0; j < E; ++j) v[E * i + j] += r[j];
  }
}

template <int BLOCK_N, Precision P, bool GNB>
__global__ void __launch_bounds__(kGemmThreads, 1) gemm_tc_kernel(const __grid_constant__ GemmParams p) {
  static_assert(!(GNB && P == kTF32), "the GroupNorm-backward epilogue is built for bf16 / split-bf16 operands");
  using Cfg = GemmCfg<BLOCK_N, GNB>;
  constexpr int kParts = parts(P);
  const int NA = p.n_aslots, NB = p.n_bslots;
  const uint32_t a_slot = (uint32_t)p.a_slot_bytes, b_slot = (uint32_t)p.b_slot_bytes;
  extern __shared__ uint8_t smem_raw[];
  uint8_t* smem = reinterpret_cast<uint8_t*>((reinterpret_cast<uintptr_t>(smem_raw) + 1023) & ~uintptr_t(1023));
  float* s_acc = reinterpret_cast<float*>(smem + NA * p.a_slot_bytes + NB * p.b_slot_bytes);
  float* s_stats = s_acc + Cfg::kAccFloats;
  uint64_t* bars = reinterpret_cast<uint64_t*>(s_stats + Cfg::kStatsFloats);

  const uint32_t a_ring = smem_u32(smem), b_ring = a_ring + NA * a_slot;
  const uint32_t a_full = smem_u32(bars), a_empty = a_full + 8 * kMaxSlots;
  const uint32_t b_full = a_empty + 8 * kMaxSlots, b_empty = b_full + 8 * kMaxSlots;

  const int warp = __shfl_sync(0xffffffffu, (int)(threadIdx.x >> 5), 0), lane = threadIdx.x & 31;

  if (warp == 0 && lane == 0) {
    for (int i = 0; i < kMaxAMaps; ++i) tma_prefetch_desc(&p.amap[i]);
    tma_prefetch_desc(&p.bmap);
  }
  if (warp == 1 && lane == 0) {
    for (int i = 0; i < NA; ++i) { mbar_init(a_full + 8 * i, 1); mbar_init(a_empty + 8 * i, 2); }
    for (int i = 0; i < NB; ++i) { mbar_init(b_full + 8 * i, 1); mbar_init(b_empty + 8 * i, 2); }
    fence_barrier_init();
    fence_proxy_async();
  }
  __syncthreads();

  const int tiles_m = p.tx * p.ty * p.tz * p.tb;
  const int splits = p.splits > 1 ? p.splits : 1;
  const int total_tiles = tiles_m * p.n_tiles_n * splits;
  const int first_tile = (int)blockIdx.x;
  const int tile_step = (int)gridDim.x;

  auto split_range = [&](int item, int& lo, int& hi) {
    const int sidx = item % splits;
    lo = (int)((long long)p.total_groups * sidx / splits);
    hi = (int)((long long)p.total_groups * (sidx + 1) / splits);
  };
  int mt_of_tile = 0;
  auto decode = [&](int tile, int& x0, int& y0, int& z0, int& b0, int& n0) {
    tile /= splits;
    int nt = tile % p.n_tiles_n;
    int mt = tile / p.n_tiles_n;
    mt_of_tile = mt;
    n0 = nt * BLOCK_N;
    int bt = 0;
    if (p.batch_fastest) { bt = mt % p.tb; mt /= p.tb; }
    int xt = mt % p.tx; mt /= p.tx;
    int yt = mt % p.ty; mt /= p.ty;
    int zt = mt % p.tz; mt /= p.tz;
    if (!p.batch_fastest) bt = mt;
    x0 = xt * p.bx; y0 = yt * p.by; z0 = zt * p.bz; b0 = bt * p.bb;
  };

  if (warp < 4) {
    setmaxnreg_dec<kRegsProducer>();
    if (warp == 0) {
      uint32_t as = 0, aph = 0, bs = 0, bph = 0;
      for (int tile = first_tile; tile < total_tiles; tile += tile_step) {
        int x0, y0, z0, b0, n0;
        decode(tile, x0, y0, z0, b0, n0);
        int kcol = 0, l = 0, gi = 0, g_lo, g_hi;
        split_range(tile, g_lo, g_hi);
        const int bcoord = p.b_batched ? b0 : 0;
        for (int sg = 0; sg < p.n_segs; ++sg) {
          const GemmSeg& seg = p.segs[sg];
          for (int g = 0; g < seg.n_groups; ++g, ++gi) {
            if (gi < g_lo || gi >= g_hi) {
              kcol += seg.nk * p.b_kstep;
              ++l;
              continue;
            }
            const uint4 raw = __ldg(reinterpret_cast<const uint4*>(p.loads + l));
            const LoadEntry& en = reinterpret_cast<const LoadEntry&>(raw);
            mbar_wait(a_empty + 8 * as, aph ^ 1);
            if (elect_one()) {
              const uint32_t abase = a_ring + as * a_slot, bar = a_full + 8 * as;
              mbar_expect_tx(bar, kParts * seg.a_bytes);
              tma_load_5d(&p.amap[en.tmap], bar, abase, en.c0, x0 + en.dx, y0 + en.dy, z0 + en.dz, b0);
              if constexpr (P == kBF16X3) tma_load_5d(&p.amap[en.tmap_lo], bar, abase + seg.a_stride, en.c0, x0 + en.dx, y0 + en.dy, z0 + en.dz, b0);
            }
            __syncwarp();
            if (++as == (uint32_t)NA) { as = 0; aph ^= 1; }
            int kc = (P == kBF16X3 && p.b_explicit_k) ? (int)en.wc0 : kcol;
            for (int j = 0; j < seg.nk; ++j) {
              mbar_wait(b_empty + 8 * bs, bph ^ 1);
              if (elect_one()) {
                const uint32_t bbase = b_ring + bs * b_slot, bar = b_full + 8 * bs;
                mbar_expect_tx(bar, kParts * Cfg::kBTileBytes);
                tma_load_3d(&p.bmap, bar, bbase, kc, n0, bcoord);
                if constexpr (P == kBF16X3) tma_load_3d(&p.bmap, bar, bbase + Cfg::kBTileBytes, kc + p.b_lo_k, n0, bcoord);
              }
              __syncwarp();
              kc += p.b_kstep;
              if (++bs == (uint32_t)NB) { bs = 0; bph ^= 1; }
            }
            kcol += seg.nk * p.b_kstep;
            ++l;
          }
        }
      }
    }
  } else {
    setmaxnreg_inc<kRegsConsumer>();
    const int wg = (warp - 4) >> 2;
    const int wt = threadIdx.x & 127;
    const int q = warp & 3;
    const int half = (warp - 4) >> 2;
    constexpr int kChunks = BLOCK_N / 32;
    constexpr int kChunkStep = kChunks >= 2 ? 2 : 1;
    const int row = q * 32 + lane;
    const int et = threadIdx.x - 128;
    const int rows_per_b = p.bx * p.by * p.bz;
    const int seg = row / rows_per_b;
    int it = 0;
    int staged_n0 = -1, staged_b0 = -1, bias_buf = 0;
    int want_cols = 0;
    if constexpr (GNB) {
      want_cols = (p.stats != nullptr || p.gnb_part != nullptr) ? 1 : 0;
      asm volatile("" : "+r"(want_cols));
    }
    uint32_t as = 0, aph = 0, bs = 0, bph = 0;
    for (int tile = first_tile; tile < total_tiles; tile += tile_step, ++it) {
      const int vit = it;
      constexpr int kAccRegs = kParts * BLOCK_N / 2;
      float acc[kAccRegs];
      float (&acc_hi)[BLOCK_N / 2] = *reinterpret_cast<float (*)[BLOCK_N / 2]>(acc);
#pragma unroll
      for (int i = 0; i < kAccRegs; ++i) acc[i] = 0.f;
      {
        int gi = 0, g_lo, g_hi;
        split_range(tile, g_lo, g_hi);
        int prev_b = -1, prev_a = -1;
        const uint32_t a_row0 = (uint32_t)wg * 64 * kRowBytes;
        for (int sg = 0; sg < p.n_segs; ++sg) {
          const GemmSeg& sgm = p.segs[sg];
          for (int g = 0; g < sgm.n_groups; ++g, ++gi) {
            if (gi < g_lo || gi >= g_hi) continue;
            mbar_wait(a_full + 8 * as, aph);
            const uint32_t abase = a_ring + as * a_slot + a_row0;
            for (int j = 0; j < sgm.nk; ++j) {
              mbar_wait(b_full + 8 * bs, bph);
              const uint64_t ad = kdesc(abase + j * sgm.jbytes);
              const uint64_t bd = kdesc(b_ring + bs * b_slot);
              wgmma_fence();
              if constexpr (P == kBF16X3) {
                const uint64_t adl = kdesc(abase + sgm.a_stride + j * sgm.jbytes);
#pragma unroll
                for (int k = 0; k < kRowBytes / 32; ++k) wgmma_kmajor<2 * BLOCK_N, false>(acc, ad + 2 * k, bd + 2 * k, 1u);
                wgmma_fence();
#pragma unroll
                for (int k = 0; k < kRowBytes / 32; ++k) wgmma_kmajor<BLOCK_N, false>(acc_hi, adl + 2 * k, bd + 2 * k, 1u);
              } else {
#pragma unroll
                for (int k = 0; k < kRowBytes / 32; ++k) wgmma_kmajor<BLOCK_N, P == kTF32>(acc, ad + 2 * k, bd + 2 * k, 1u);
              }
              wgmma_commit();
              wgmma_wait<1>();
              if (wt == 0) {
                if (prev_b >= 0) mbar_arrive(b_empty + 8 * prev_b);
                if (prev_a >= 0) mbar_arrive(a_empty + 8 * prev_a);
              }
              prev_b = (int)bs;
              prev_a = j + 1 == sgm.nk ? (int)as : -1;
              if (++bs == (uint32_t)NB) { bs = 0; bph ^= 1; }
            }
            if (++as == (uint32_t)NA) { as = 0; aph ^= 1; }
          }
        }
        wgmma_wait<0>();
        fence_operands(acc);
        if (wt == 0) {
          if (prev_b >= 0) mbar_arrive(b_empty + 8 * prev_b);
          if (prev_a >= 0) mbar_arrive(a_empty + 8 * prev_a);
        }
        if constexpr (P == kBF16X3) {
#pragma unroll
          for (int i = 0; i < BLOCK_N / 2; ++i) acc[i] += acc[BLOCK_N / 2 + i];
        }
      }
      int x0, y0, z0, b0, n0;
      decode(tile, x0, y0, z0, b0, n0);
      int r = row;
      const int xl = r % p.bx; r /= p.bx;
      const int yl = r % p.by; r /= p.by;
      const int zl = r % p.bz; r /= p.bz;
      const int xg = x0 + xl, yg = y0 + yl, zg = z0 + zl, bg = b0 + r;
      const bool valid = (xg < p.X) && (yg < p.Y) && (zg < p.Z) && (bg < p.Bn);
      const long long ooff = xg * p.osx + yg * p.osy + zg * p.osz + bg * p.osb;
      const long long roff = xg * p.rsx + yg * p.rsy + zg * p.rsz + bg * p.rsb;

      constexpr int kRoundRegs = Cfg::kStageCols / 2;
      auto stage = [&]() {
        const int w4 = (warp & 3), srow = wg * 64 + w4 * 16 + (lane >> 2), scol = 2 * (lane & 3);
#pragma unroll
        for (int j = 0; j < Cfg::kStageCols / 8; ++j) {
          *reinterpret_cast<float2*>(s_acc + srow * Cfg::kAccPitch + 8 * j + scol) = make_float2(acc[4 * j], acc[4 * j + 1]);
          *reinterpret_cast<float2*>(s_acc + (srow + 8) * Cfg::kAccPitch + 8 * j + scol) = make_float2(acc[4 * j + 2], acc[4 * j + 3]);
        }
      };
      named_bar_sync(2, kEpiThreads);
      stage();
      if constexpr (Cfg::kStageRounds > 1) {
#pragma unroll
        for (int i = 0; i < kRoundRegs; ++i) acc[i] = acc[kRoundRegs + i];
      }

      const int bkey = p.rowbias ? b0 : 0;
      if (n0 != staged_n0 || bkey != staged_b0) {
        staged_n0 = n0; staged_b0 = bkey;
        bias_buf ^= 1;
        float* wb = s_stats + 16 * BLOCK_N + bias_buf * 4 * BLOCK_N;
        for (int i = et; i < p.bb * BLOCK_N; i += kEpiThreads) {
          const int sg = i / BLOCK_N, c = i % BLOCK_N;
          const int n = n0 + c, bgl = b0 + sg;
          float bv = 0.f;
          if (n < p.N) {
            if (p.bias && !p.bias_on_m) bv += __ldg(p.bias + n);
            if (p.rowbias && bgl < p.Bn) bv += __ldg(p.rowbias + static_cast<long long>(bgl) * p.rowbias_ld + n);
          }
          wb[i] = bv;
        }
      }
      const float* s_bias = s_stats + 16 * BLOCK_N + bias_buf * 4 * BLOCK_N;
      float* s_part = s_stats + (vit & 1) * 8 * BLOCK_N;
      uint4 rbuf[8];
      auto prefetch_res = [&](int ch) {
        const int nbp = n0 + ch * 32;
        if (!(p.res && valid && p.ocs == 1 && nbp + 32 <= p.N)) return;
        if constexpr (GNB) {
          const bool second = p.res1 && nbp >= p.res_c0;
          const __nv_bfloat16* base = reinterpret_cast<const __nv_bfloat16*>(second ? p.res1 : p.res);
          const long long off = second ? xg * p.r1sx + yg * p.r1sy + zg * p.r1sz + bg * p.r1sb + (nbp - p.res_c0) : roff + nbp;
          const uint4* rp = reinterpret_cast<const uint4*>(base + off);
#pragma unroll
          for (int i = 0; i < 4; ++i) rbuf[i] = __ldg(rp + i);
          if constexpr (P == kBF16X3) {
            const uint4* rl = reinterpret_cast<const uint4*>(base + off + (second ? p.res1_lo_off : p.res_lo_off));
#pragma unroll
            for (int i = 0; i < 4; ++i) rbuf[4 + i] = __ldg(rl + i);
          }
          return;
        }
        if (P == kTF32 || p.res_fp32) {
          const uint4* rp = reinterpret_cast<const uint4*>(reinterpret_cast<const float*>(p.res) + roff + nbp);
#pragma unroll
          for (int i = 0; i < 8; ++i) rbuf[i] = __ldg(rp + i);
        } else {
          const uint4* rp = reinterpret_cast<const uint4*>(reinterpret_cast<const __nv_bfloat16*>(p.res) + roff + nbp);
#pragma unroll
          for (int i = 0; i < 4; ++i) rbuf[i] = __ldg(rp + i);
          if constexpr (P == kBF16X3) {
            const uint4* rl = reinterpret_cast<const uint4*>(reinterpret_cast<const __nv_bfloat16*>(p.res) + roff + nbp + p.res_lo_off);
#pragma unroll
            for (int i = 0; i < 4; ++i) rbuf[4 + i] = __ldg(rl + i);
          }
        }
      };
      const int ch0 = kChunkStep == 2 ? half : 0;
      const bool active = kChunkStep == 2 || half == 0;
      if (active) prefetch_res(ch0);

      constexpr int kRoundChunks = Cfg::kStageCols / 32;
#pragma unroll 1
      for (int rnd = 0; rnd < Cfg::kStageRounds; ++rnd) {
        if (rnd > 0) {
          named_bar_sync(2, kEpiThreads);
          stage();
        }
        named_bar_sync(2, kEpiThreads);

#pragma unroll 1
        for (int ch = ch0 + rnd * kRoundChunks; ch < (rnd + 1) * kRoundChunks && active; ch += kChunkStep) {
          uint32_t rr[32];
          {
            const float4* src = reinterpret_cast<const float4*>(s_acc + row * Cfg::kAccPitch + (ch - rnd * kRoundChunks) * 32);
#pragma unroll
            for (int i = 0; i < 8; ++i) {
              const float4 t = src[i];
              rr[4 * i] = __float_as_uint(t.x); rr[4 * i + 1] = __float_as_uint(t.y);
              rr[4 * i + 2] = __float_as_uint(t.z); rr[4 * i + 3] = __float_as_uint(t.w);
            }
          }
          const int nb = n0 + ch * 32;
          if (nb >= p.N) continue;
          if (splits > 1) {
            if (valid) {
              float* pp = p.partial + (long long)(tile % splits) * p.split_stride + (P == kBF16X3 ? (ooff >> 1) : ooff) + nb;
              if (nb + 32 <= p.N) {
#pragma unroll
                for (int i = 0; i < 8; ++i)
                  reinterpret_cast<float4*>(pp)[i] = make_float4(__uint_as_float(rr[4 * i]), __uint_as_float(rr[4 * i + 1]),
                                                                 __uint_as_float(rr[4 * i + 2]), __uint_as_float(rr[4 * i + 3]));
              } else {
                for (int i = 0; i < 32; ++i) if (nb + i < p.N) pp[i] = __uint_as_float(rr[i]);
              }
            }
            continue;
          }
          const bool full = (nb + 32 <= p.N) && (p.ocs == 1);
          float v[32];
          const float mbias = (p.bias && p.bias_on_m && valid) ? __ldg(p.bias + xg) : 0.f;
          const float* sb = s_bias + (seg < 4 ? seg : 0) * BLOCK_N + ch * 32;
#pragma unroll
          for (int i = 0; i < 32; ++i) v[i] = __uint_as_float(rr[i]) * p.alpha + mbias + sb[i];
          float q2[GNB ? 32 : 1];
          if constexpr (GNB) {
            if (valid) {
              const float4* cc = p.gnb_c + static_cast<long long>(bg) * p.N + nb;
              unsigned long long hsh[8];
              if (p.gnb_drop_thresh > 0) {
                const unsigned long long e4 = (unsigned long long)((((static_cast<long long>(bg) * p.Z + zg) * p.Y + yg) * p.X + xg) * p.N + nb) >> 2;
#pragma unroll
                for (int i = 0; i < 8; ++i) hsh[i] = drop_hash64(p.gnb_seed, e4 + i);
              }
#pragma unroll
              for (int i = 0; i < 32; ++i) {
                const float4 kc = __ldg(cc + i);
                const __nv_bfloat16 xb = reinterpret_cast<const __nv_bfloat16*>(rbuf)[i];
                float xv = __bfloat162float(xb);
                if constexpr (P == kBF16X3) xv += __bfloat162float(reinterpret_cast<const __nv_bfloat16*>(rbuf + 4)[i]);
                float d = v[i];
                if (p.gnb_drop_thresh > 0) {
                  const unsigned r16 = (unsigned)((hsh[i >> 2] >> (16 * (i & 3))) & 0xFFFFu);
                  d = r16 >= (unsigned)p.gnb_drop_thresh ? d * p.gnb_drop_scale : 0.f;
                }
                if (p.gnb_silu) {
                  const float h = fmaf(xv, kc.x, kc.y);
                  d *= P == kBF16X3 ? dsilu_ex2_half(h) : dsilu_tanh_half(h);
                }
                v[i] = d;
                q2[i] = d * fmaf(xv, kc.z, kc.w);
              }
            } else {
#pragma unroll
              for (int i = 0; i < 32; ++i) q2[i] = 0.f;
            }
          }
          if (!GNB && p.res && valid) {
            if (P == kTF32 || p.res_fp32) {
              if (full) {
                add_res_chunk<kTF32>(rbuf, v);
              } else {
                const float* rp = reinterpret_cast<const float*>(p.res) + roff + nb;
                for (int i = 0; i < 32; ++i) if (nb + i < p.N) v[i] += rp[i];
              }
            } else {
              if (full) {
                add_res_chunk<P>(rbuf, v);
              } else {
                const ActElem<P>* rp = reinterpret_cast<const ActElem<P>*>(p.res) + roff + nb;
                for (int i = 0; i < 32; ++i) if (nb + i < p.N) v[i] += load_split<P>(rp + i, p.res_lo_off);
              }
            }
          }
          if (ch + kChunkStep < kChunks) prefetch_res(ch + kChunkStep);
          if (valid) {
            if (p.out_fp32) {
              float* op = reinterpret_cast<float*>(p.out) + ooff + nb;
              if (full) {
#pragma unroll
                for (int i = 0; i < 8; ++i) reinterpret_cast<float4*>(op)[i] = make_float4(v[4 * i], v[4 * i + 1], v[4 * i + 2], v[4 * i + 3]);
              } else {
                for (int i = 0; i < 32; ++i) if (nb + i < p.N) op[i * p.ocs] = v[i];
              }
            } else {
              ActElem<P>* op = reinterpret_cast<ActElem<P>*>(p.out) + ooff + nb;
              if (full) {
                constexpr int E = kVecElems<P>;
#pragma unroll
                for (int i = 0; i < 32 / E; ++i) store_vec<P>(op + E * i, p.out_lo_off * (long long)sizeof(ActElem<P>), v + E * i);
              } else {
                for (int i = 0; i < 32; ++i) if (nb + i < p.N) store_split<P>(op + i * p.ocs, p.out_lo_off, v[i]);
              }
            }
          }
          if (GNB ? (want_cols != 0) : (p.stats != nullptr)) {
            float s[32], ss[32];
#pragma unroll
            for (int i = 0; i < 32; ++i) {
              const float t = valid ? v[i] : 0.f;
              s[i] = t; ss[i] = GNB ? q2[GNB ? i : 0] : t * t;
            }
            colsum_butterfly<16>(s, ss, lane);
            s_part[(q * 2 + 0) * BLOCK_N + ch * 32 + lane] = s[0];
            s_part[(q * 2 + 1) * BLOCK_N + ch * 32 + lane] = ss[0];
          }
        }
      }
      if constexpr (GNB) {
        if (p.gnb_part && splits == 1) {
          named_bar_sync(1, kEpiThreads);
          const int warps_per_seg = rows_per_b >= 128 ? 4 : rows_per_b / 32;
          for (int i = et; i < p.bb * BLOCK_N; i += kEpiThreads) {
            const int sg = i / BLOCK_N, c = i % BLOCK_N;
            const int n = n0 + c;
            if (mt_of_tile < tiles_m && n < p.N) {
              float ts = 0.f, tq = 0.f;
              for (int w = sg * warps_per_seg; w < (sg + 1) * warps_per_seg; ++w) {
                ts += s_part[(w * 2 + 0) * BLOCK_N + c];
                tq += s_part[(w * 2 + 1) * BLOCK_N + c];
              }
              float* dst = p.gnb_part + ((static_cast<long long>(mt_of_tile) * p.bb + sg) * p.N + n) * 2;
              dst[0] = ts; dst[1] = tq;
            }
          }
        }
      }
      if (!GNB && p.stats && splits == 1) {
        named_bar_sync(1, kEpiThreads);
        const int warps_per_seg = rows_per_b >= 128 ? 4 : rows_per_b / 32;
        for (int i0 = 0; i0 < p.bb * BLOCK_N; i0 += kEpiThreads) {
          const int i = i0 + et;
          const int sg = i / BLOCK_N, c = i % BLOCK_N;
          const int bgl = b0 + sg, n = n0 + c;
          if (i < p.bb * BLOCK_N && bgl < p.Bn && n < p.N) {
            float ts = 0.f, tq = 0.f;
            for (int w = sg * warps_per_seg; w < (sg + 1) * warps_per_seg; ++w) {
              ts += s_part[(w * 2 + 0) * BLOCK_N + c];
              tq += s_part[(w * 2 + 1) * BLOCK_N + c];
            }
            long long* dst = p.stats + (static_cast<long long>(bgl) * p.N + n) * kStatWords;
            stat_add(dst, ts);
            stat_add(dst + 2, tq);
          }
        }
      }
    }
  }
}

}
```

meshdiffusion_b200/diffusion/models/ddpm.py:

```python
import ctypes
import math

import numpy as np
import torch
import torch.nn as nn

from ... import _native
from . import utils


PRECISIONS = {"bf16": 0, "tf32": 1, "bf16x3": 2}
TRAIN_PRECISIONS = ("bf16", "bf16x3")


def arch_from_config(config):
    is128 = config.model.name.startswith("ddpm_res128")
    return dict(
        image_size=int(config.data.image_size), nf=int(config.model.nf),
        ch_mult=tuple(int(c) for c in config.model.ch_mult), num_res_blocks=int(config.model.num_res_blocks),
        attn_resolutions=tuple(int(r) for r in config.model.attn_resolutions),
        num_channels=int(config.data.num_channels), stem_ksize=5 if is128 else 3, use_pos_bias=not is128,
        level0_blocks=2 if is128 else int(config.model.num_res_blocks),
    )


def _config_c(arch, max_batch, precision, training=False):
    c = _native.UNetConfigC()
    c.image_size, c.nf, c.n_levels = arch["image_size"], arch["nf"], len(arch["ch_mult"])
    for i, v in enumerate(arch["ch_mult"]):
        c.ch_mult[i] = v
    c.num_res_blocks, c.level0_blocks = arch["num_res_blocks"], arch["level0_blocks"]
    c.n_attn = len(arch["attn_resolutions"])
    for i, v in enumerate(arch["attn_resolutions"]):
        c.attn_resolutions[i] = v
    c.num_channels, c.stem_ksize = arch["num_channels"], arch["stem_ksize"]
    c.use_pos_bias = 1 if arch["use_pos_bias"] else 0
    c.max_batch, c.precision = max_batch, PRECISIONS[precision]
    c.training = 1 if training else 0
    return c


def param_table(arch):
    L = _native.lib()
    h = ctypes.c_void_p()
    cfg = _config_c(arch, 1, "bf16")
    _native.check(L.mdb_unet_create_dry(ctypes.byref(cfg), ctypes.byref(h)))
    try:
        out = []
        for i in range(L.mdb_unet_num_params(h)):
            name, numel, nd = ctypes.c_char_p(), ctypes.c_longlong(), ctypes.c_int()
            shape = (ctypes.c_longlong * 8)()
            _native.check(L.mdb_unet_param_info(h, i, ctypes.byref(name), ctypes.byref(numel), ctypes.byref(nd), shape))
            out.append((name.value.decode(), tuple(int(shape[j]) for j in range(nd.value))))
        return out
    finally:
        L.mdb_unet_destroy(h)


def variance_scaling_uniform(shape, scale=1.0, generator=None):
    scale = 1e-10 if scale == 0 else scale
    receptive = 1
    for d in shape[2:]:
        receptive *= d
    fan_in, fan_out = shape[1] * receptive, shape[0] * receptive
    bound = math.sqrt(3.0 * scale / ((fan_in + fan_out) / 2.0))
    return (torch.rand(shape, generator=generator) * 2.0 - 1.0) * bound


def make_grad_buckets(entries, total_numel, bucket_bytes):
    buckets, hi, ready = [], total_numel, 0
    for off, numel, rdy in sorted(entries, reverse=True):
        ready = max(ready, rdy)
        if (hi - off) * 4 >= bucket_bytes:
            buckets.append((ready, off, hi))
            hi, ready = off, 0
    if hi > 0:
        buckets.append((ready, 0, hi))
    buckets.sort()
    return buckets


class _ScoreNetFn(torch.autograd.Function):

    @staticmethod
    def forward(ctx, net, x, labels, *params):
        out = net._train_forward(x, labels, net._diff_precision(), net.dropout if net.training else 0.0)
        ctx.net = net
        ctx.save_for_backward(x, labels)
        return out

    @staticmethod
    def backward(ctx, dout):
        x, labels = ctx.saved_tensors
        dx = ctx.net._train_backward(x, labels, dout, want_x=ctx.needs_input_grad[1], want_params=any(ctx.needs_input_grad[3:]))
        return (None, dx, None) + (None,) * len(ctx.net._trainable)


class _Scope(nn.Module):
    """Plain container so dotted parameter names become nested state-dict keys."""


class ScoreNet(nn.Module):
    def __init__(self, config):
        super().__init__()
        self.arch = arch_from_config(config)
        self.precision = str(config.model.get("compute_dtype", "bf16x3")) if hasattr(config.model, "get") else "bf16x3"
        if self.precision not in PRECISIONS:
            raise ValueError("config.model.compute_dtype must be 'bf16', 'tf32' or 'bf16x3'")
        training = getattr(config, "training", None)
        self.train_precision = str(training.get("compute_dtype", "bf16")) if hasattr(training, "get") else "bf16"
        if self.train_precision not in TRAIN_PRECISIONS:
            raise ValueError("config.training.compute_dtype must be 'bf16' or 'bf16x3'")
        self.max_batch = int(config.model.get("engine_max_batch", 0) or 0) if hasattr(config.model, "get") else 0
        self.scale_by_sigma = bool(config.model.scale_by_sigma)
        self.dropout = float(config.model.get("dropout", 0.0)) if hasattr(config.model, "get") else 0.0
        self._train_handle, self._train_batch, self._train_synced = None, 0, None
        self._xgrad_handle, self._xgrad_batch, self._xgrad_synced = None, 0, None
        self._flat_grad, self._drop_calls, self._pending = None, 0, None
        self.reduce_in_backward = False
        self.grad_overlap = bool(config.model.get("grad_overlap", True)) if hasattr(config.model, "get") else True
        self.bucket_bytes = int(config.model.get("grad_bucket_mb", 64)) << 20 if hasattr(config.model, "get") else 64 << 20
        self._buckets, self._pending_reduce, self._side_stream = None, None, None
        self.register_buffer("sigmas", torch.tensor(utils.get_sigmas(config)))
        self._names = []
        head_idx = None
        table = param_table(self.arch)
        for name, _ in table:
            if name.startswith("all_modules."):
                head_idx = max(head_idx or 0, int(name.split(".")[1]))
        def ref_order(item):
            n = item[0]
            if n == "coords": return (0, 0)
            if n == "mask": return (1, 0)
            if n.startswith("pos_layer."): return (2, 0)
            if n.startswith("mask_layer."): return (3, 0)
            return (4, int(n.split(".")[1]))
        for name, shape in sorted(table, key=ref_order):
            self._register(name, self._initial_value(name, shape, head_idx), trainable=name not in ("mask", "coords"))
        self._handle = None
        self._engine_batch = 0
        self._synced = None
        self._trainable = [n for n in self._names if n not in ("mask", "coords")]

    def _initial_value(self, name, shape, head_idx):
        leaf = name.split(".")[-1]
        if name == "mask" or name == "coords":
            return torch.zeros(shape)
        if leaf in ("bias", "b"):
            return torch.zeros(shape)
        if "GroupNorm" in name or name == f"all_modules.{head_idx - 1}.weight":
            return torch.ones(shape)
        if leaf == "W":
            return variance_scaling_uniform(shape, 0.0 if name.endswith("NIN_3.W") else 0.1)
        zero_init = name.endswith("Conv_1.weight") or name == f"all_modules.{head_idx}.weight"
        return variance_scaling_uniform(shape, 0.0 if zero_init else 1.0)

    def _register(self, dotted, value, trainable):
        parts = dotted.split(".")
        node = self
        for p in parts[:-1]:
            if not hasattr(node, p):
                node.add_module(p, _Scope())
            node = getattr(node, p)
        node.register_parameter(parts[-1], nn.Parameter(value, requires_grad=trainable))
        self._names.append(dotted)

    def _param(self, dotted):
        node = self
        for p in dotted.split("."):
            node = getattr(node, p)
        return node

    def _ensure_engine(self, batch, device):
        L = _native.lib()
        if self._handle is not None and batch <= self._engine_batch:
            return
        if device.type != "cuda":
            raise _native.NativeError("the score network runs only on a CUDA (sm_90a) device; there is no CPU path")
        self.release_engine()
        mb = max(batch, self.max_batch)
        cfg = _config_c(self.arch, mb, self.precision)
        h = ctypes.c_void_p()
        with torch.cuda.device(device):
            _native.check(L.mdb_unet_create(ctypes.byref(cfg), ctypes.byref(h)))
        self._handle, self._engine_batch, self._synced = h, mb, None

    def release_engine(self):
        if self._handle is not None:
            _native.lib().mdb_unet_destroy(self._handle)
            self._handle = None
        if getattr(self, "_train_handle", None) is not None:
            _native.lib().mdb_unet_destroy(self._train_handle)
            self._train_handle = None
        if getattr(self, "_xgrad_handle", None) is not None:
            _native.lib().mdb_unet_destroy(self._xgrad_handle)
            self._xgrad_handle = None

    def _ensure_train_engine(self, batch, device):
        L = _native.lib()
        if self._train_handle is not None and batch <= self._train_batch:
            return
        if device.type != "cuda":
            raise _native.NativeError("the score network trains only on a CUDA (sm_90a) device; there is no CPU path")
        if self._train_handle is not None:
            L.mdb_unet_destroy(self._train_handle)
            self._train_handle = None
        cfg = _config_c(self.arch, batch, self.train_precision, training=True)
        h = ctypes.c_void_p()
        with torch.cuda.device(device):
            _native.check(L.mdb_unet_create(ctypes.byref(cfg), ctypes.byref(h)))
        self._train_handle, self._train_batch, self._train_synced = h, batch, None
        self._ensure_flat_grad(h, device)
        self._buckets = None

    def _ensure_flat_grad(self, h, device):
        L = _native.lib()
        numel = ctypes.c_longlong()
        _native.check(L.mdb_unet_train_info(h, None, None, ctypes.byref(numel)))
        if self._flat_grad is None or self._flat_grad.numel() != numel.value or self._flat_grad.device != device:
            self._flat_grad = torch.zeros(numel.value, dtype=torch.float32, device=device)
            self._grad_views = {}
            for n in self._trainable:
                off = ctypes.c_longlong()
                _native.check(L.mdb_unet_grad_offset(h, n.encode(), ctypes.byref(off)))
                p = self._param(n)
                self._grad_views[n] = self._flat_grad[off.value:off.value + p.numel()].view(p.shape)

    def _diff_precision(self):
        if self.training:
            return self.train_precision
        if self.precision not in TRAIN_PRECISIONS:
            raise ValueError(f"input gradients through model.eval() run the training plan, which takes config.model.compute_dtype "
                             f"'bf16' or 'bf16x3', not '{self.precision}'")
        return self.precision

    def _diff_engine(self, precision, batch, device):
        if precision == self.train_precision:
            self._ensure_train_engine(batch, device)
            self._train_synced = self._push_parameters(self._train_handle, self._train_synced)
            return self._train_handle
        L = _native.lib()
        if self._xgrad_handle is None or batch > self._xgrad_batch:
            if device.type != "cuda":
                raise _native.NativeError("the score network runs only on a CUDA (sm_90a) device; there is no CPU path")
            if self._xgrad_handle is not None:
                L.mdb_unet_destroy(self._xgrad_handle)
                self._xgrad_handle = None
            cfg = _config_c(self.arch, batch, precision, training=True)
            h = ctypes.c_void_p()
            with torch.cuda.device(device):
                _native.check(L.mdb_unet_create(ctypes.byref(cfg), ctypes.byref(h)))
            self._xgrad_handle, self._xgrad_batch, self._xgrad_synced = h, batch, None
        self._xgrad_synced = self._push_parameters(self._xgrad_handle, self._xgrad_synced)
        return self._xgrad_handle

    def _grad_buckets(self):
        if self._buckets is not None:
            return self._buckets
        L = _native.lib()
        entries = []
        for n in self._names:
            off, rdy = ctypes.c_longlong(), ctypes.c_int()
            _native.check(L.mdb_unet_grad_offset(self._train_handle, n.encode(), ctypes.byref(off)))
            _native.check(L.mdb_unet_grad_ready(self._train_handle, n.encode(), ctypes.byref(rdy)))
            entries.append((off.value, self._param(n).numel(), rdy.value))
        self._buckets = make_grad_buckets(entries, self._flat_grad.numel(), self.bucket_bytes)
        return self._buckets

    def _backward_with_overlapped_allreduce(self, dout, B, accumulate):
        import torch.distributed as dist
        L = _native.lib()
        buckets = self._grad_buckets()
        if self._side_stream is None:
            self._side_stream = torch.cuda.Stream(device=self._flat_grad.device)
            self._events = [torch.cuda.Event() for _ in buckets]
            for e in self._events:
                e.record()
        n = len(buckets)
        steps = (ctypes.c_int * n)(*[b[0] for b in buckets])
        handles = (ctypes.c_void_p * n)(*[e.cuda_event for e in self._events])
        _native.check(L.mdb_unet_backward_marked(self._train_handle, _native.ptr(dout), _native.ptr(self._flat_grad), self._flat_grad.numel(),
                                                 B, 1 if accumulate else 0, steps, handles, n, _native.current_stream()))
        works = []
        with torch.cuda.stream(self._side_stream):
            for (rdy, lo, hi), ev in zip(buckets, self._events):
                self._side_stream.wait_event(ev)
                works.append(dist.all_reduce(self._flat_grad[lo:hi], op=dist.ReduceOp.AVG, async_op=True))
        self._pending_reduce = works

    def _push_parameters(self, handle, synced):
        L = _native.lib()
        fp = self._fingerprints()
        changed = None if synced is None else (fp != synced).nonzero().flatten().tolist()
        if changed is not None and not changed:
            return fp
        stream = _native.current_stream()
        self._upload(handle, range(len(self._names)) if changed is None else changed, stream)
        torch.cuda.current_stream().synchronize()
        _native.check(L.mdb_unet_commit(handle, stream))
        return fp

    def _upload(self, handle, indices, stream):
        L = _native.lib()
        indices = tuple(indices)
        params = [self._param(self._names[i]) for i in indices]
        bulk = [k for k, p in enumerate(params) if p.is_cuda and p.dtype == torch.float32 and p.is_contiguous()]
        if bulk:
            key = (tuple(indices[k] for k in bulk), tuple(params[k].data_ptr() for k in bulk))
            cache = getattr(self, "_upload_cache", None)
            if cache is None or cache[0] != key:
                m = len(bulk)
                names = (ctypes.c_char_p * m)(*[self._names[indices[k]].encode() for k in bulk])
                srcs = (ctypes.c_void_p * m)(*key[1])
                numels = (ctypes.c_longlong * m)(*[params[k].numel() for k in bulk])
                cache = self._upload_cache = (key, m, names, srcs, numels)
            _native.check(L.mdb_unet_set_params(handle, cache[1], cache[2], cache[3], cache[4], stream))
        done = set(bulk)
        for k, p in enumerate(params):
            if k in done:
                continue
            src = p.detach().float().contiguous()
            _native.check(L.mdb_unet_set_param(handle, self._names[indices[k]].encode(), _native.ptr(src), src.numel(),
                                               1 if src.is_cuda else 0, stream))
            if src.is_cuda:
                src.record_stream(torch.cuda.current_stream())

    def _train_forward(self, x, labels, precision, p):
        L = _native.lib()
        B = x.shape[0]
        with torch.cuda.device(x.device):
            h = self._diff_engine(precision, B, x.device)
            self._drop_calls += 1
            seed = (torch.initial_seed() * 1000003 + self._drop_calls) & 0xFFFFFFFFFFFFFFFF
            _native.check(L.mdb_unet_set_dropout(h, p, seed))
            out = torch.empty_like(x)
            _native.check(L.mdb_unet_forward(h, _native.ptr(x), _native.ptr(labels), _native.ptr(out), B, _native.current_stream()))
        self._pending = (h.value, x.data_ptr(), B)
        return out

    def _train_backward(self, x, labels, dout, want_x=False, want_params=True):
        L = _native.lib()
        B = x.shape[0]
        if self._pending is None or self._pending[1:] != (x.data_ptr(), B):
            raise _native.NativeError("backward() must follow the forward() it differentiates: the engine keeps the "
                                      "activations of one forward pass at a time")
        h = ctypes.c_void_p(self._pending[0])
        dx = torch.empty_like(x) if want_x else None
        if not want_params:
            with torch.cuda.device(x.device):
                _native.check(L.mdb_unet_backward_input(h, _native.ptr(dout.float().contiguous()), _native.ptr(dx), None, 0, B, 0,
                                                        _native.current_stream()))
            self._pending = None
            return dx
        self._ensure_flat_grad(h, x.device)

        def backward(grads, accumulate):
            if dx is None:
                _native.check(L.mdb_unet_backward(h, _native.ptr(dout), _native.ptr(grads), grads.numel(), B, accumulate,
                                                  _native.current_stream()))
            else:
                _native.check(L.mdb_unet_backward_input(h, _native.ptr(dout), _native.ptr(dx), _native.ptr(grads), grads.numel(), B,
                                                        accumulate, _native.current_stream()))
        params = [self._param(n) for n in self._trainable]
        none = [p.grad is None for p in params]
        ours = [p.grad is not None and p.grad.data_ptr() == self._grad_views[n].data_ptr() for p, n in zip(params, self._trainable)]
        dout = dout.float().contiguous()
        import torch.distributed as dist
        overlap = (self.reduce_in_backward and self.grad_overlap and dist.is_available() and dist.is_initialized() and dist.get_world_size() > 1
                   and dist.get_backend() == "nccl" and dx is None and h.value == getattr(self._train_handle, "value", None))
        with torch.cuda.device(x.device):
            if all(none) or all(ours):
                if overlap:
                    self._backward_with_overlapped_allreduce(dout, B, accumulate=not all(none))
                else:
                    backward(self._flat_grad, 0 if all(none) else 1)
                if all(none):
                    for p, n in zip(params, self._trainable):
                        p.grad = self._grad_views[n]
            else:
                tmp = torch.zeros_like(self._flat_grad)
                backward(tmp, 0)
                for p, n in zip(params, self._trainable):
                    v = self._grad_views[n]
                    g = tmp[v.storage_offset():v.storage_offset() + v.numel()].view(p.shape)
                    p.grad = g.clone() if p.grad is None else p.grad + g
        self._pending = None
        return dx

    def allreduce_grads(self):
        import torch.distributed as dist
        if self._flat_grad is None or not (dist.is_available() and dist.is_initialized()) or dist.get_world_size() == 1:
            return
        if self._pending_reduce is not None:
            for w in self._pending_reduce:
                w.wait()
            self._pending_reduce = None
            return
        dist.all_reduce(self._flat_grad, op=dist.ReduceOp.SUM)
        self._flat_grad.mul_(1.0 / dist.get_world_size())

    def __del__(self):
        try:
            self.release_engine()
        except Exception:
            pass

    def _fingerprints(self):
        L = _native.lib()
        params = [self._param(n) for n in self._names]
        key = tuple(p.data_ptr() for p in params)
        if getattr(self, "_fp_key", None) != key:
            dev = params[0].device
            self._fp_ptrs = torch.tensor(key, dtype=torch.int64, device=dev)
            self._fp_numels = torch.tensor([p.numel() for p in params], dtype=torch.int64, device=dev)
            self._fp_out = torch.empty(len(params), dtype=torch.int64, device=dev)
            self._fp_key = key
        _native.check(L.mdb_fingerprint(_native.ptr(self._fp_ptrs), _native.ptr(self._fp_numels), len(params),
                                        _native.ptr(self._fp_out), _native.current_stream()))
        return self._fp_out.cpu()

    def frozen(self):
        net = self

        class _Frozen:
            def __enter__(self_inner):
                net.sync_parameters()
                net._frozen = True

            def __exit__(self_inner, *exc):
                net._frozen = False

        return _Frozen()

    def sync_parameters(self, force=False):
        L = _native.lib()
        if getattr(self, "_frozen", False) and not force:
            return
        fp = self._fingerprints()
        changed = None if (force or self._synced is None) else (fp != self._synced).nonzero().flatten().tolist()
        if changed is not None and not changed:
            return
        stream = _native.current_stream()
        self._upload(self._handle, range(len(self._names)) if changed is None else changed, stream)
        torch.cuda.current_stream().synchronize()
        _native.check(L.mdb_unet_commit(self._handle, stream))
        self._synced = fp

    def score_vjp(self, x, labels, v):
        if self.scale_by_sigma:
            raise ValueError("score_vjp differentiates the raw network output (scale_by_sigma=False)")
        if not x.is_cuda:
            raise _native.NativeError("the score network runs only on a CUDA (sm_90a) device; there is no CPU path")
        precision = self._diff_precision()
        x = x.float().contiguous()
        labels = labels.to(device=x.device, dtype=torch.float32).contiguous()
        out = self._train_forward(x, labels, precision, 0.0)
        return out, self._train_backward(x, labels, v, want_x=True, want_params=False)

    def forward(self, x, labels):
        input_grad = not self.training and torch.is_grad_enabled() and x.requires_grad
        if input_grad:
            self._diff_precision()
        if not x.is_cuda:
            raise _native.NativeError("the score network runs only on a CUDA (sm_90a) device; there is no CPU path")
        L = _native.lib()
        x = x.float().contiguous()
        labels = labels.to(device=x.device, dtype=torch.float32).contiguous()
        B = x.shape[0]
        if input_grad or (self.training and torch.is_grad_enabled() and any(self._param(n).requires_grad for n in self._trainable)):
            out = _ScoreNetFn.apply(self, x, labels, *[self._param(n) for n in self._trainable])
            if self.scale_by_sigma:
                out = out / self.sigmas.to(out.device)[labels.long(), None, None, None, None].float()
            return out
        with torch.cuda.device(x.device):
            self._ensure_engine(B, x.device)
            self.sync_parameters()
            out = torch.empty_like(x)
            _native.check(L.mdb_unet_forward(self._handle, _native.ptr(x), _native.ptr(labels), _native.ptr(out), B,
                                             _native.current_stream()))
        if self.scale_by_sigma:
            out = out / self.sigmas.to(out.device)[labels.long(), None, None, None, None].float()
        return out

    def engine_info(self):
        L = _native.lib()
        fl, ar, ng, ns = ctypes.c_double(), ctypes.c_longlong(), ctypes.c_int(), ctypes.c_int()
        _native.check(L.mdb_unet_info(self._handle, ctypes.byref(fl), ctypes.byref(ar), ctypes.byref(ng), ctypes.byref(ns)))
        return dict(flops_per_sample=fl.value, arena_bytes=ar.value, gemm_launches=ng.value, steps=ns.value,
                    max_batch=self._engine_batch, precision=self.precision)

    def gemm_ops(self):
        L = _native.lib()
        rows = []
        for i in range(self.engine_info()["gemm_launches"]):
            name, fl, fb = ctypes.c_char_p(), ctypes.c_double(), ctypes.c_double()
            _native.check(L.mdb_unet_gemm_ops(self._handle, i, ctypes.byref(name), ctypes.byref(fl), ctypes.byref(fb)))
            rows.append((name.value.decode(), fl.value, fb.value))
        return rows

    def gemm_slots(self):
        L = _native.lib()
        rows = []
        for i in range(self.engine_info()["gemm_launches"]):
            a, b, sm = ctypes.c_int(), ctypes.c_int(), ctypes.c_int()
            _native.check(L.mdb_unet_gemm_slots(self._handle, i, ctypes.byref(a), ctypes.byref(b), ctypes.byref(sm)))
            rows.append((a.value, b.value, sm.value))
        return rows

    def gemm_tiles(self):
        L = _native.lib()
        rows = []
        for i in range(self.engine_info()["gemm_launches"]):
            v = [ctypes.c_int() for _ in range(5)]
            _native.check(L.mdb_unet_gemm_tiles(self._handle, i, *[ctypes.byref(x) for x in v]))
            rows.append(tuple(x.value for x in v))
        return rows

    def profile(self, x, labels):
        L = _native.lib()
        B = x.shape[0]
        self._ensure_engine(B, x.device)
        self.sync_parameters()
        out = torch.empty_like(x)
        names = ctypes.create_string_buffer(1 << 16)
        ms = (ctypes.c_float * 1024)()
        n = ctypes.c_int()
        _native.check(L.mdb_unet_profile(self._handle, _native.ptr(x), _native.ptr(labels), _native.ptr(out), B,
                                         _native.current_stream(), names, len(names), ms, 1024, ctypes.byref(n)))
        return list(zip(names.value.decode().strip().split("\n"), [ms[i] for i in range(n.value)]))


@utils.register_model(name="ddpm_res64")
class DDPMRes64(ScoreNet):
    pass


@utils.register_model(name="ddpm_res128")
class DDPMRes128(ScoreNet):
    pass


utils.register_model(DDPMRes128, name="ddpm_res128_v2")
```

Baseline: 36.39.

## Add handoff epilogue mode overlapping accumulator drain with next tile's MMA

Adds a second GEMM epilogue variant in which the consumer warpgroups stage accumulators into shared-memory handoff buffers, guarded by mbarriers, and a separate set of epilogue warps performs bias, residual, store and stats work. This lets the math warps start the next tile's main loop sooner. The mode is chosen per GEMM when ksteps per split reaches a threshold, and an environment variable can override the choice. It costs extra barrier traffic, shared memory for the buffers and more kernel template instantiations.

```diff
diff --git a/include/meshdiff_b200.h b/include/meshdiff_b200.h
--- a/include/meshdiff_b200.h
+++ b/include/meshdiff_b200.h
@@ -43,6 +43,7 @@
 int mdb_unet_info(mdb_unet* net, double* flops_per_sample, long long* arena_bytes, int* n_gemm_launches, int* n_steps);
 int mdb_unet_gemm_ops(mdb_unet* net, int i, const char** name, double* flops, double* fill_bytes);
 int mdb_unet_gemm_slots(mdb_unet* net, int i, int* a_slots, int* b_slots, int* smem_bytes);
+int mdb_unet_gemm_epilogue(mdb_unet* net, int i, int* handoff);
 int mdb_unet_gemm_tiles(mdb_unet* net, int i, int* work_items, int* splits, int* ksteps, int* entry_ksteps, int* block_n);
 int mdb_unet_profile(mdb_unet* net, const float* x, const float* labels, float* out, int batch, void* stream,
                      char* names_buf, int names_len, float* ms, int max_steps, int* n_steps);
diff --git a/meshdiffusion_b200/_native.py b/meshdiffusion_b200/_native.py
--- a/meshdiffusion_b200/_native.py
+++ b/meshdiffusion_b200/_native.py
@@ -61,6 +61,7 @@
     "mdb_unet_info": (_i, [_vp, ctypes.POINTER(_d), ctypes.POINTER(_ll), ctypes.POINTER(_i), ctypes.POINTER(_i)]),
     "mdb_unet_gemm_ops": (_i, [_vp, _i, ctypes.POINTER(ctypes.c_char_p), ctypes.POINTER(_d), ctypes.POINTER(_d)]),
     "mdb_unet_gemm_slots": (_i, [_vp, _i, ctypes.POINTER(_i), ctypes.POINTER(_i), ctypes.POINTER(_i)]),
+    "mdb_unet_gemm_epilogue": (_i, [_vp, _i, ctypes.POINTER(_i)]),
     "mdb_unet_gemm_tiles": (_i, [_vp, _i, ctypes.POINTER(_i), ctypes.POINTER(_i), ctypes.POINTER(_i), ctypes.POINTER(_i),
                                  ctypes.POINTER(_i)]),
     "mdb_unet_profile": (_i, [_vp, _vp, _vp, _vp, _i, _vp, ctypes.c_char_p, _i, ctypes.POINTER(_f), _i, ctypes.POINTER(_i)]),
diff --git a/meshdiffusion_b200/csrc/api.cu b/meshdiffusion_b200/csrc/api.cu
--- a/meshdiffusion_b200/csrc/api.cu
+++ b/meshdiffusion_b200/csrc/api.cu
@@ -126,6 +126,13 @@
   if (a_slots) *a_slots = a;
   if (b_slots) *b_slots = b;
   if (smem_bytes) *smem_bytes = sm;
+  MDB_API_END
+}
+
+int mdb_unet_gemm_epilogue(mdb_unet* n, int i, int* handoff) {
+  MDB_API_BEGIN
+  if (i < 0 || i >= n->net->num_gemm_launches()) throw std::runtime_error("mdb: GEMM launch index out of range");
+  if (handoff) *handoff = n->net->gemm(i).epilogue() == kHandoff ? 1 : 0;
   MDB_API_END
 }
 
diff --git a/meshdiffusion_b200/csrc/gemm_host.cu b/meshdiffusion_b200/csrc/gemm_host.cu
--- a/meshdiffusion_b200/csrc/gemm_host.cu
+++ b/meshdiffusion_b200/csrc/gemm_host.cu
@@ -43,10 +43,10 @@
   }
 }
 
-template <int BN, Precision P, bool GNB>
+template <int BN, Precision P, bool GNB, EpiMode E>
 static void launch_impl(const GemmParams& p, int grid, int smem, cudaStream_t stream) {
   static bool configured[64] = {};
-  auto kern = gemm_tc_kernel<BN, P, GNB>;
+  auto kern = gemm_tc_kernel<BN, P, GNB, E>;
   int dev = 0;
   MDB_CUDA_CHECK(cudaGetDevice(&dev));
   if (dev >= 64 || !configured[dev]) {
@@ -61,22 +61,34 @@
   void (*launch)(const GemmParams&, int grid, int smem, cudaStream_t);
   int fixed_bytes;
 };
-template <int BN, Precision P, bool GNB>
-static GemmVariant variant() { return {launch_impl<BN, P, GNB>, GemmCfg<BN, GNB>::kFixedBytes}; }
+template <int BN, Precision P, bool GNB, EpiMode E = kInline>
+static GemmVariant variant() { return {launch_impl<BN, P, GNB, E>, GemmCfg<BN, GNB>::kFixedBytes}; }
+template <int BN, Precision P>
+static GemmVariant variant(EpiMode e) { return e == kHandoff ? variant<BN, P, false, kHandoff>() : variant<BN, P, false>(); }
 template <int BN>
-static GemmVariant variant(Precision prec, bool gnb) {
+static GemmVariant variant(Precision prec, bool gnb, EpiMode e) {
   if (gnb) {
     if (prec == kTF32) throw std::runtime_error("mdb: the GroupNorm-backward epilogue is built for bf16 / split-bf16 operands");
     return prec == kBF16X3 ? variant<BN, kBF16X3, true>() : variant<BN, kBF16, true>();
   }
-  return prec == kTF32 ? variant<BN, kTF32, false>() : prec == kBF16X3 ? variant<BN, kBF16X3, false>() : variant<BN, kBF16, false>();
-}
-static GemmVariant gemm_variant(int block_n, Precision prec, bool gnb) {
-  return block_n == 32 ? variant<32>(prec, gnb) : variant<128>(prec, gnb);
+  return prec == kTF32 ? variant<BN, kTF32>(e) : prec == kBF16X3 ? variant<BN, kBF16X3>(e) : variant<BN, kBF16>(e);
+}
+static GemmVariant gemm_variant(int block_n, Precision prec, bool gnb, EpiMode e) {
+  return block_n == 32 ? variant<32>(prec, gnb, e) : variant<128>(prec, gnb, e);
+}
+
+EpiMode GemmOp::epilogue() const {
+  if (gnb) return kInline;
+  if (const char* e = getenv("MDB_GEMM_EPILOGUE")) {
+    if (!strcmp(e, "inline")) return kInline;
+    if (!strcmp(e, "handoff")) return kHandoff;
+  }
+  const int s = p.splits > 1 ? p.splits : 1;
+  return ksteps / s >= kHandoffMinKsteps ? kHandoff : kInline;
 }
 
 int GemmOp::pick_slots(GemmParams& q) const {
-  const int fixed = gemm_variant(block_n, prec, gnb).fixed_bytes;
+  const int fixed = gemm_variant(block_n, prec, gnb, epilogue()).fixed_bytes;
   const int budget = kMaxDynSmem - fixed;
   q.a_slot_bytes = (a_slot_need + 1023) / 1024 * 1024;
   q.b_slot_bytes = parts(prec) * block_n * kRowBytes;
@@ -526,7 +538,7 @@
     if (p.splits > 1) throw std::runtime_error("mdb: GroupNorm-backward epilogue: no split-K");
     p.gnb_drop_thresh = rt_drop_thresh; p.gnb_drop_scale = rt_drop_scale; p.gnb_seed = rt_seed;
   }
-  gemm_variant(block_n, prec, gnb).launch(p, grid, smem, stream);
+  gemm_variant(block_n, prec, gnb, epilogue()).launch(p, grid, smem, stream);
   if (p.splits > 1) {
     SplitReduceArgs a{};
     a.partial = p.partial; a.split_stride = p.split_stride; a.splits = p.splits;
diff --git a/meshdiffusion_b200/csrc/gemm_host.h b/meshdiffusion_b200/csrc/gemm_host.h
--- a/meshdiffusion_b200/csrc/gemm_host.h
+++ b/meshdiffusion_b200/csrc/gemm_host.h
@@ -108,6 +108,7 @@
   void launch(cudaStream_t stream, int B = -1, void* out_override = nullptr) const;
   double fill_bytes(int B = -1) const;
   void slots(int& a_slots, int& b_slots, int& smem_bytes) const;
+  EpiMode epilogue() const;
 
  private:
   Geometry geo{};
@@ -121,6 +122,8 @@
   MapDesc b_desc(void* ptr, long long K, int N, int batch, long long row_stride_bytes, long long batch_stride_bytes) const;
 };
 
+constexpr int kHandoffMinKsteps = 16;
+
 int sm_count();
 constexpr int kPlanSMs = 132;
 void encode_map(CUtensorMap* m, Precision prec, const MapDesc& d);
diff --git a/meshdiffusion_b200/csrc/gemm_tc.cuh b/meshdiffusion_b200/csrc/gemm_tc.cuh
--- a/meshdiffusion_b200/csrc/gemm_tc.cuh
+++ b/meshdiffusion_b200/csrc/gemm_tc.cuh
@@ -13,6 +13,9 @@
 constexpr int kMaxAMaps = 16;
 constexpr int kGemmThreads = 384;
 constexpr int kEpiThreads = 256;
+constexpr int kHandoffEpiWarps = 3;
+
+enum EpiMode : int { kInline = 0, kHandoff = 1 };
 
 struct __align__(16) LoadEntry {
   uint8_t tmap;
@@ -97,6 +100,8 @@
   static_assert(kStageRounds <= 2, "the epilogue stages at most two rounds");
   static constexpr int kAccPitch = kStageCols + 4;
   static constexpr int kAccFloats = kBlockM * kAccPitch;
+  static constexpr int kHandoffCol = 36;
+  static constexpr int kHandoffBufs = kAccPitch >= kHandoffCol + 32 ? 2 : 1;
   static constexpr int kFixedBytes = 1024 + kAccFloats * 4 + kStatsFloats * 4 + 4 * kMaxSlots * 8;
 };
 constexpr int kRegsProducer = 40, kRegsConsumer = 232;
@@ -130,9 +135,209 @@
   }
 }
 
+template <int BLOCK_N>
+__device__ __forceinline__ void stage_bias(const GemmParams& p, float* wb, int n0, int b0, int t, int nthreads) {
+  for (int i = t; i < p.bb * BLOCK_N; i += nthreads) {
+    const int sg = i / BLOCK_N, c = i % BLOCK_N;
+    const int n = n0 + c, bgl = b0 + sg;
+    float bv = 0.f;
+    if (n < p.N) {
+      if (p.bias && !p.bias_on_m) bv += __ldg(p.bias + n);
+      if (p.rowbias && bgl < p.Bn) bv += __ldg(p.rowbias + static_cast<long long>(bgl) * p.rowbias_ld + n);
+    }
+    wb[i] = bv;
+  }
+}
+
+template <int BLOCK_N>
+__device__ __forceinline__ void column_stats(const GemmParams& p, const float* s_part, int n0, int b0, int t, int nthreads) {
+  const int rows_per_b = p.bx * p.by * p.bz;
+  const int warps_per_seg = rows_per_b >= 128 ? 4 : rows_per_b / 32;
+  for (int i0 = 0; i0 < p.bb * BLOCK_N; i0 += nthreads) {
+    const int i = i0 + t;
+    const int sg = i / BLOCK_N, c = i % BLOCK_N;
+    const int bgl = b0 + sg, n = n0 + c;
+    if (i < p.bb * BLOCK_N && bgl < p.Bn && n < p.N) {
+      float ts = 0.f, tq = 0.f;
+      for (int w = sg * warps_per_seg; w < (sg + 1) * warps_per_seg; ++w) {
+        ts += s_part[(w * 2 + 0) * BLOCK_N + c];
+        tq += s_part[(w * 2 + 1) * BLOCK_N + c];
+      }
+      long long* dst = p.stats + (static_cast<long long>(bgl) * p.N + n) * kStatWords;
+      stat_add(dst, ts);
+      stat_add(dst + 2, tq);
+    }
+  }
+}
+
 template <int BLOCK_N, Precision P, bool GNB>
+struct EpiRow {
+  const GemmParams& p;
+  int tile, splits, n0;
+  int xg, yg, zg, bg;
+  bool valid;
+  long long ooff, roff;
+  uint4 rbuf[8];
+
+  __device__ __forceinline__ EpiRow(const GemmParams& p_, int tile_, int splits_, int row, int x0, int y0, int z0, int b0,
+                                    int n0_)
+      : p(p_), tile(tile_), splits(splits_), n0(n0_) {
+    int r = row;
+    const int xl = r % p.bx; r /= p.bx;
+    const int yl = r % p.by; r /= p.by;
+    const int zl = r % p.bz; r /= p.bz;
+    xg = x0 + xl; yg = y0 + yl; zg = z0 + zl; bg = b0 + r;
+    valid = (xg < p.X) && (yg < p.Y) && (zg < p.Z) && (bg < p.Bn);
+    ooff = xg * p.osx + yg * p.osy + zg * p.osz + bg * p.osb;
+    roff = xg * p.rsx + yg * p.rsy + zg * p.rsz + bg * p.rsb;
+  }
+
+  __device__ __forceinline__ void prefetch_res(int ch) {
+    const int nbp = n0 + ch * 32;
+    if (!(p.res && valid && p.ocs == 1 && nbp + 32 <= p.N)) return;
+    if constexpr (GNB) {
+      const bool second = p.res1 && nbp >= p.res_c0;
+      const __nv_bfloat16* base = reinterpret_cast<const __nv_bfloat16*>(second ? p.res1 : p.res);
+      const long long off = second ? xg * p.r1sx + yg * p.r1sy + zg * p.r1sz + bg * p.r1sb + (nbp - p.res_c0) : roff + nbp;
+      const uint4* rp = reinterpret_cast<const uint4*>(base + off);
+#pragma unroll
+      for (int i = 0; i < 4; ++i) rbuf[i] = __ldg(rp + i);
+      if constexpr (P == kBF16X3) {
+        const uint4* rl = reinterpret_cast<const uint4*>(base + off + (second ? p.res1_lo_off : p.res_lo_off));
+#pragma unroll
+        for (int i = 0; i < 4; ++i) rbuf[4 + i] = __ldg(rl + i);
+      }
+      return;
+    }
+    if (P == kTF32 || p.res_fp32) {
+      const uint4* rp = reinterpret_cast<const uint4*>(reinterpret_cast<const float*>(p.res) + roff + nbp);
+#pragma unroll
+      for (int i = 0; i < 8; ++i) rbuf[i] = __ldg(rp + i);
+    } else {
+      const uint4* rp = reinterpret_cast<const uint4*>(reinterpret_cast<const __nv_bfloat16*>(p.res) + roff + nbp);
+#pragma unroll
+      for (int i = 0; i < 4; ++i) rbuf[i] = __ldg(rp + i);
+      if constexpr (P == kBF16X3) {
+        const uint4* rl = reinterpret_cast<const uint4*>(reinterpret_cast<const __nv_bfloat16*>(p.res) + roff + nbp + p.res_lo_off);
+#pragma unroll
+        for (int i = 0; i < 4; ++i) rbuf[4 + i] = __ldg(rl + i);
+      }
+    }
+  }
+
+  __device__ __forceinline__ void chunk(int ch, int next_ch, const uint32_t (&rr)[32], const float* s_bias, int seg,
+                                        float* s_part, int q, int lane, int want_cols) {
+    const int nb = n0 + ch * 32;
+    if (nb >= p.N) return;
+    if (splits > 1) {
+      if (valid) {
+        float* pp = p.partial + (long long)(tile % splits) * p.split_stride + (P == kBF16X3 ? (ooff >> 1) : ooff) + nb;
+        if (nb + 32 <= p.N) {
+#pragma unroll
+          for (int i = 0; i < 8; ++i)
+            reinterpret_cast<float4*>(pp)[i] = make_float4(__uint_as_float(rr[4 * i]), __uint_as_float(rr[4 * i + 1]),
+                                                           __uint_as_float(rr[4 * i + 2]), __uint_as_float(rr[4 * i + 3]));
+        } else {
+          for (int i = 0; i < 32; ++i) if (nb + i < p.N) pp[i] = __uint_as_float(rr[i]);
+        }
+      }
+      return;
+    }
+    const bool full = (nb + 32 <= p.N) && (p.ocs == 1);
+    float v[32];
+    const float mbias = (p.bias && p.bias_on_m && valid) ? __ldg(p.bias + xg) : 0.f;
+    const float* sb = s_bias + (seg < 4 ? seg : 0) * BLOCK_N + ch * 32;
+#pragma unroll
+    for (int i = 0; i < 32; ++i) v[i] = __uint_as_float(rr[i]) * p.alpha + mbias + sb[i];
+    float q2[GNB ? 32 : 1];
+    if constexpr (GNB) {
+      if (valid) {
+        const float4* cc = p.gnb_c + static_cast<long long>(bg) * p.N + nb;
+        unsigned long long hsh[8];
+        if (p.gnb_drop_thresh > 0) {
+          const unsigned long long e4 = (unsigned long long)((((static_cast<long long>(bg) * p.Z + zg) * p.Y + yg) * p.X + xg) * p.N + nb) >> 2;
+#pragma unroll
+          for (int i = 0; i < 8; ++i) hsh[i] = drop_hash64(p.gnb_seed, e4 + i);
+        }
+#pragma unroll
+        for (int i = 0; i < 32; ++i) {
+          const float4 kc = __ldg(cc + i);
+          const __nv_bfloat16 xb = reinterpret_cast<const __nv_bfloat16*>(rbuf)[i];
+          float xv = __bfloat162float(xb);
+          if constexpr (P == kBF16X3) xv += __bfloat162float(reinterpret_cast<const __nv_bfloat16*>(rbuf + 4)[i]);
+          float d = v[i];
+          if (p.gnb_drop_thresh > 0) {
+            const unsigned r16 = (unsigned)((hsh[i >> 2] >> (16 * (i & 3))) & 0xFFFFu);
+            d = r16 >= (unsigned)p.gnb_drop_thresh ? d * p.gnb_drop_scale : 0.f;
+          }
+          if (p.gnb_silu) {
+            const float h = fmaf(xv, kc.x, kc.y);
+            d *= P == kBF16X3 ? dsilu_ex2_half(h) : dsilu_tanh_half(h);
+          }
+          v[i] = d;
+          q2[i] = d * fmaf(xv, kc.z, kc.w);
+        }
+      } else {
+#pragma unroll
+        for (int i = 0; i < 32; ++i) q2[i] = 0.f;
+      }
+    }
+    if (!GNB && p.res && valid) {
+      if (P == kTF32 || p.res_fp32) {
+        if (full) {
+          add_res_chunk<kTF32>(rbuf, v);
+        } else {
+          const float* rp = reinterpret_cast<const float*>(p.res) + roff + nb;
+          for (int i = 0; i < 32; ++i) if (nb + i < p.N) v[i] += rp[i];
+        }
+      } else {
+        if (full) {
+          add_res_chunk<P>(rbuf, v);
+        } else {
+          const ActElem<P>* rp = reinterpret_cast<const ActElem<P>*>(p.res) + roff + nb;
+          for (int i = 0; i < 32; ++i) if (nb + i < p.N) v[i] += load_split<P>(rp + i, p.res_lo_off);
+        }
+      }
+    }
+    if (next_ch >= 0) prefetch_res(next_ch);
+    if (valid) {
+      if (p.out_fp32) {
+        float* op = reinterpret_cast<float*>(p.out) + ooff + nb;
+        if (full) {
+#pragma unroll
+          for (int i = 0; i < 8; ++i) reinterpret_cast<float4*>(op)[i] = make_float4(v[4 * i], v[4 * i + 1], v[4 * i + 2], v[4 * i + 3]);
+        } else {
+          for (int i = 0; i < 32; ++i) if (nb + i < p.N) op[i * p.ocs] = v[i];
+        }
+      } else {
+        ActElem<P>* op = reinterpret_cast<ActElem<P>*>(p.out) + ooff + nb;
+        if (full) {
+          constexpr int E = kVecElems<P>;
+#pragma unroll
+          for (int i = 0; i < 32 / E; ++i) store_vec<P>(op + E * i, p.out_lo_off * (long long)sizeof(ActElem<P>), v + E * i);
+        } else {
+          for (int i = 0; i < 32; ++i) if (nb + i < p.N) store_split<P>(op + i * p.ocs, p.out_lo_off, v[i]);
+        }
+      }
+    }
+    if (GNB ? (want_cols != 0) : (p.stats != nullptr)) {
+      float s[32], ss[32];
+#pragma unroll
+      for (int i = 0; i < 32; ++i) {
+        const float t = valid ? v[i] : 0.f;
+        s[i] = t; ss[i] = GNB ? q2[GNB ? i : 0] : t * t;
+      }
+      colsum_butterfly<16>(s, ss, lane);
+      s_part[(q * 2 + 0) * BLOCK_N + ch * 32 + lane] = s[0];
+      s_part[(q * 2 + 1) * BLOCK_N + ch * 32 + lane] = ss[0];
+    }
+  }
+};
+
+template <int BLOCK_N, Precision P, bool GNB, EpiMode E = kInline>
 __global__ void __launch_bounds__(kGemmThreads, 1) gemm_tc_kernel(const __grid_constant__ GemmParams p) {
   static_assert(!(GNB && P == kTF32), "the GroupNorm-backward epilogue is built for bf16 / split-bf16 operands");
+  static_assert(!(GNB && E == kHandoff), "the GroupNorm-backward epilogue runs inline");
   using Cfg = GemmCfg<BLOCK_N, GNB>;
   constexpr int kParts = parts(P);
   const int NA = p.n_aslots, NB = p.n_bslots;
@@ -146,6 +351,8 @@
   const uint32_t a_ring = smem_u32(smem), b_ring = a_ring + NA * a_slot;
   const uint32_t a_full = smem_u32(bars), a_empty = a_full + 8 * kMaxSlots;
   const uint32_t b_full = a_empty + 8 * kMaxSlots, b_empty = b_full + 8 * kMaxSlots;
+  auto h_full = [&](int b) { return smem_u32(s_acc + b * Cfg::kAccPitch + 32); };
+  auto h_empty = [&](int b) { return smem_u32(s_acc + b * Cfg::kAccPitch + 34); };
 
   const int warp = __shfl_sync(0xffffffffu, (int)(threadIdx.x >> 5), 0), lane = threadIdx.x & 31;
 
@@ -156,6 +363,9 @@
   if (warp == 1 && lane == 0) {
     for (int i = 0; i < NA; ++i) { mbar_init(a_full + 8 * i, 1); mbar_init(a_empty + 8 * i, 2); }
     for (int i = 0; i < NB; ++i) { mbar_init(b_full + 8 * i, 1); mbar_init(b_empty + 8 * i, 2); }
+    if constexpr (E == kHandoff) {
+      for (int b = 0; b < Cfg::kHandoffBufs; ++b) { mbar_init(h_full(b), kEpiThreads); mbar_init(h_empty(b), 128); }
+    }
     fence_barrier_init();
     fence_proxy_async();
   }
@@ -189,7 +399,7 @@
   };
 
   if (warp < 4) {
-    setmaxnreg_dec<kRegsProducer>();
+    if constexpr (E == kInline) setmaxnreg_dec<kRegsProducer>();
     if (warp == 0) {
       uint32_t as = 0, aph = 0, bs = 0, bph = 0;
       for (int tile = first_tile; tile < total_tiles; tile += tile_step) {
@@ -236,8 +446,54 @@
         }
       }
     }
+    if constexpr (E == kHandoff) {
+      if (warp > 0) {
+        const int e = warp - 1, t = threadIdx.x - 32;
+        constexpr int kChunks = BLOCK_N / 32, kBufs = Cfg::kHandoffBufs;
+        constexpr int kEwgThreads = kHandoffEpiWarps * 32;
+        const int rows_per_b = p.bx * p.by * p.bz;
+        int staged_n0 = -1, staged_b0 = -1, bias_buf = 0;
+        int it = 0;
+        for (int tile = first_tile; tile < total_tiles; tile += tile_step, ++it) {
+          int x0, y0, z0, b0, n0;
+          decode(tile, x0, y0, z0, b0, n0);
+          const int bkey = p.rowbias ? b0 : 0;
+          if (n0 != staged_n0 || bkey != staged_b0) {
+            staged_n0 = n0; staged_b0 = bkey;
+            bias_buf ^= 1;
+            stage_bias<BLOCK_N>(p, s_stats + 16 * BLOCK_N + bias_buf * 4 * BLOCK_N, n0, b0, t, kEwgThreads);
+          }
+          const float* s_bias = s_stats + 16 * BLOCK_N + bias_buf * 4 * BLOCK_N;
+          float* s_part = s_stats + (it & 1) * 8 * BLOCK_N;
+          named_bar_sync(2, kEwgThreads);
+#pragma unroll 1
+          for (int u = e; u < 4 * kChunks; u += kHandoffEpiWarps) {
+            const int ch = u >> 2, q = u & 3, row = q * 32 + lane;
+            EpiRow<BLOCK_N, P, false> er(p, tile, splits, row, x0, y0, z0, b0, n0);
+            er.prefetch_res(ch);
+            const int b = ch % kBufs;
+            const uint32_t use = (uint32_t)(it * (kChunks / kBufs) + ch / kBufs);
+            mbar_wait(h_full(b), use & 1);
+            uint32_t rr[32];
+            const float4* src = reinterpret_cast<const float4*>(s_acc + row * Cfg::kAccPitch + b * Cfg::kHandoffCol);
+#pragma unroll
+            for (int i = 0; i < 8; ++i) {
+              const float4 v4 = src[i];
+              rr[4 * i] = __float_as_uint(v4.x); rr[4 * i + 1] = __float_as_uint(v4.y);
+              rr[4 * i + 2] = __float_as_uint(v4.z); rr[4 * i + 3] = __float_as_uint(v4.w);
+            }
+            mbar_arrive(h_empty(b));
+            er.chunk(ch, -1, rr, s_bias, row / rows_per_b, s_part, q, lane, 0);
+          }
+          if (p.stats && splits == 1) {
+            named_bar_sync(1, kEwgThreads);
+            column_stats<BLOCK_N>(p, s_part, n0, b0, t, kEwgThreads);
+          }
+        }
+      }
+    }
   } else {
-    setmaxnreg_inc<kRegsConsumer>();
+    if constexpr (E == kInline) setmaxnreg_inc<kRegsConsumer>();
     const int wg = (warp - 4) >> 2;
     const int wt = threadIdx.x & 127;
     const int q = warp & 3;
@@ -314,251 +570,314 @@
           for (int i = 0; i < BLOCK_N / 2; ++i) acc[i] += acc[BLOCK_N / 2 + i];
         }
       }
-      int x0, y0, z0, b0, n0;
-      decode(tile, x0, y0, z0, b0, n0);
-      int r = row;
-      const int xl = r % p.bx; r /= p.bx;
-      const int yl = r % p.by; r /= p.by;
-      const int zl = r % p.bz; r /= p.bz;
-      const int xg = x0 + xl, yg = y0 + yl, zg = z0 + zl, bg = b0 + r;
-      const bool valid = (xg < p.X) && (yg < p.Y) && (zg < p.Z) && (bg < p.Bn);
-      const long long ooff = xg * p.osx + yg * p.osy + zg * p.osz + bg * p.osb;
-      const long long roff = xg * p.rsx + yg * p.rsy + zg * p.rsz + bg * p.rsb;
-
-      constexpr int kRoundRegs = Cfg::kStageCols / 2;
-      auto stage = [&]() {
-        const int w4 = (warp & 3), srow = wg * 64 + w4 * 16 + (lane >> 2), scol = 2 * (lane & 3);
-#pragma unroll
-        for (int j = 0; j < Cfg::kStageCols / 8; ++j) {
-          *reinterpret_cast<float2*>(s_acc + srow * Cfg::kAccPitch + 8 * j + scol) = make_float2(acc[4 * j], acc[4 * j + 1]);
-          *reinterpret_cast<float2*>(s_acc + (srow + 8) * Cfg::kAccPitch + 8 * j + scol) = make_float2(acc[4 * j + 2], acc[4 * j + 3]);
-        }
-      };
-      named_bar_sync(2, kEpiThreads);
-      stage();
-      if constexpr (Cfg::kStageRounds > 1) {
-#pragma unroll
-        for (int i = 0; i < kRoundRegs; ++i) acc[i] = acc[kRoundRegs + i];
-      }
-
-      const int bkey = p.rowbias ? b0 : 0;
-      if (n0 != staged_n0 || bkey != staged_b0) {
-        staged_n0 = n0; staged_b0 = bkey;
-        bias_buf ^= 1;
-        float* wb = s_stats + 16 * BLOCK_N + bias_buf * 4 * BLOCK_N;
-        for (int i = et; i < p.bb * BLOCK_N; i += kEpiThreads) {
-          const int sg = i / BLOCK_N, c = i % BLOCK_N;
-          const int n = n0 + c, bgl = b0 + sg;
-          float bv = 0.f;
-          if (n < p.N) {
-            if (p.bias && !p.bias_on_m) bv += __ldg(p.bias + n);
-            if (p.rowbias && bgl < p.Bn) bv += __ldg(p.rowbias + static_cast<long long>(bgl) * p.rowbias_ld + n);
-          }
-          wb[i] = bv;
-        }
-      }
-      const float* s_bias = s_stats + 16 * BLOCK_N + bias_buf * 4 * BLOCK_N;
-      float* s_part = s_stats + (vit & 1) * 8 * BLOCK_N;
-      uint4 rbuf[8];
-      auto prefetch_res = [&](int ch) {
-        const int nbp = n0 + ch * 32;
-        if (!(p.res && valid && p.ocs == 1 && nbp + 32 <= p.N)) return;
-        if constexpr (GNB) {
-          const bool second = p.res1 && nbp >= p.res_c0;
-          const __nv_bfloat16* base = reinterpret_cast<const __nv_bfloat16*>(second ? p.res1 : p.res);
-          const long long off = second ? xg * p.r1sx + yg * p.r1sy + zg * p.r1sz + bg * p.r1sb + (nbp - p.res_c0) : roff + nbp;
-          const uint4* rp = reinterpret_cast<const uint4*>(base + off);
-#pragma unroll
-          for (int i = 0; i < 4; ++i) rbuf[i] = __ldg(rp + i);
-          if constexpr (P == kBF16X3) {
-            const uint4* rl = reinterpret_cast<const uint4*>(base + off + (second ? p.res1_lo_off : p.res_lo_off));
-#pragma unroll
-            for (int i = 0; i < 4; ++i) rbuf[4 + i] = __ldg(rl + i);
-          }
-          return;
-        }
-        if (P == kTF32 || p.res_fp32) {
-          const uint4* rp = reinterpret_cast<const uint4*>(reinterpret_cast<const float*>(p.res) + roff + nbp);
-#pragma unroll
-          for (int i = 0; i < 8; ++i) rbuf[i] = __ldg(rp + i);
-        } else {
-          const uint4* rp = reinterpret_cast<const uint4*>(reinterpret_cast<const __nv_bfloat16*>(p.res) + roff + nbp);
-#pragma unroll
-          for (int i = 0; i < 4; ++i) rbuf[i] = __ldg(rp + i);
-          if constexpr (P == kBF16X3) {
-            const uint4* rl = reinterpret_cast<const uint4*>(reinterpret_cast<const __nv_bfloat16*>(p.res) + roff + nbp + p.res_lo_off);
-#pragma unroll
-            for (int i = 0; i < 4; ++i) rbuf[4 + i] = __ldg(rl + i);
-          }
-        }
-      };
-      const int ch0 = kChunkStep == 2 ? half : 0;
-      const bool active = kChunkStep == 2 || half == 0;
-      if (active) prefetch_res(ch0);
-
-      constexpr int kRoundChunks = Cfg::kStageCols / 32;
-#pragma unroll 1
-      for (int rnd = 0; rnd < Cfg::kStageRounds; ++rnd) {
-        if (rnd > 0) {
-          named_bar_sync(2, kEpiThreads);
-          stage();
-        }
+      if constexpr (E == kHandoff) {
+        constexpr int kBufs = Cfg::kHandoffBufs;
+        const int srow = wg * 64 + (warp & 3) * 16 + (lane >> 2), scol = 2 * (lane & 3);
+#pragma unroll
+        for (int c = 0; c < kChunks; ++c) {
+          const int b = c % kBufs;
+          const uint32_t use = (uint32_t)(it * (kChunks / kBufs) + c / kBufs);
+          mbar_wait(h_empty(b), (use & 1) ^ 1);
+          float* dst = s_acc + b * Cfg::kHandoffCol + scol;
+#pragma unroll
+          for (int j = 0; j < 4; ++j) {
+            const int a = 16 * c + 4 * j;
+            *reinterpret_cast<float2*>(dst + srow * Cfg::kAccPitch + 8 * j) = make_float2(acc[a], acc[a + 1]);
+            *reinterpret_cast<float2*>(dst + (srow + 8) * Cfg::kAccPitch + 8 * j) = make_float2(acc[a + 2], acc[a + 3]);
+          }
+          mbar_arrive(h_full(b));
+        }
+        continue;
+      }
+      if constexpr (GNB) {
+        int x0, y0, z0, b0, n0;
+        decode(tile, x0, y0, z0, b0, n0);
+        int r = row;
+        const int xl = r % p.bx; r /= p.bx;
+        const int yl = r % p.by; r /= p.by;
+        const int zl = r % p.bz; r /= p.bz;
+        const int xg = x0 + xl, yg = y0 + yl, zg = z0 + zl, bg = b0 + r;
+        const bool valid = (xg < p.X) && (yg < p.Y) && (zg < p.Z) && (bg < p.Bn);
+        const long long ooff = xg * p.osx + yg * p.osy + zg * p.osz + bg * p.osb;
+        const long long roff = xg * p.rsx + yg * p.rsy + zg * p.rsz + bg * p.rsb;
+
+        constexpr int kRoundRegs = Cfg::kStageCols / 2;
+        auto stage = [&]() {
+          const int w4 = (warp & 3), srow = wg * 64 + w4 * 16 + (lane >> 2), scol = 2 * (lane & 3);
+#pragma unroll
+          for (int j = 0; j < Cfg::kStageCols / 8; ++j) {
+            *reinterpret_cast<float2*>(s_acc + srow * Cfg::kAccPitch + 8 * j + scol) = make_float2(acc[4 * j], acc[4 * j + 1]);
+            *reinterpret_cast<float2*>(s_acc + (srow + 8) * Cfg::kAccPitch + 8 * j + scol) = make_float2(acc[4 * j + 2], acc[4 * j + 3]);
+          }
+        };
         named_bar_sync(2, kEpiThreads);
-
-#pragma unroll 1
-        for (int ch = ch0 + rnd * kRoundChunks; ch < (rnd + 1) * kRoundChunks && active; ch += kChunkStep) {
-          uint32_t rr[32];
-          {
-            const float4* src = reinterpret_cast<const float4*>(s_acc + row * Cfg::kAccPitch + (ch - rnd * kRoundChunks) * 32);
-#pragma unroll
-            for (int i = 0; i < 8; ++i) {
-              const float4 t = src[i];
-              rr[4 * i] = __float_as_uint(t.x); rr[4 * i + 1] = __float_as_uint(t.y);
-              rr[4 * i + 2] = __float_as_uint(t.z); rr[4 * i + 3] = __float_as_uint(t.w);
-            }
-          }
-          const int nb = n0 + ch * 32;
-          if (nb >= p.N) continue;
-          if (splits > 1) {
-            if (valid) {
-              float* pp = p.partial + (long long)(tile % splits) * p.split_stride + (P == kBF16X3 ? (ooff >> 1) : ooff) + nb;
-              if (nb + 32 <= p.N) {
-#pragma unroll
-                for (int i = 0; i < 8; ++i)
-                  reinterpret_cast<float4*>(pp)[i] = make_float4(__uint_as_float(rr[4 * i]), __uint_as_float(rr[4 * i + 1]),
-                                                                 __uint_as_float(rr[4 * i + 2]), __uint_as_float(rr[4 * i + 3]));
-              } else {
-                for (int i = 0; i < 32; ++i) if (nb + i < p.N) pp[i] = __uint_as_float(rr[i]);
-              }
-            }
-            continue;
-          }
-          const bool full = (nb + 32 <= p.N) && (p.ocs == 1);
-          float v[32];
-          const float mbias = (p.bias && p.bias_on_m && valid) ? __ldg(p.bias + xg) : 0.f;
-          const float* sb = s_bias + (seg < 4 ? seg : 0) * BLOCK_N + ch * 32;
-#pragma unroll
-          for (int i = 0; i < 32; ++i) v[i] = __uint_as_float(rr[i]) * p.alpha + mbias + sb[i];
-          float q2[GNB ? 32 : 1];
-          if constexpr (GNB) {
-            if (valid) {
-              const float4* cc = p.gnb_c + static_cast<long long>(bg) * p.N + nb;
-              unsigned long long hsh[8];
-              if (p.gnb_drop_thresh > 0) {
-                const unsigned long long e4 = (unsigned long long)((((static_cast<long long>(bg) * p.Z + zg) * p.Y + yg) * p.X + xg) * p.N + nb) >> 2;
-#pragma unroll
-                for (int i = 0; i < 8; ++i) hsh[i] = drop_hash64(p.gnb_seed, e4 + i);
-              }
-#pragma unroll
-              for (int i = 0; i < 32; ++i) {
-                const float4 kc = __ldg(cc + i);
-                const __nv_bfloat16 xb = reinterpret_cast<const __nv_bfloat16*>(rbuf)[i];
-                float xv = __bfloat162float(xb);
-                if constexpr (P == kBF16X3) xv += __bfloat162float(reinterpret_cast<const __nv_bfloat16*>(rbuf + 4)[i]);
-                float d = v[i];
-                if (p.gnb_drop_thresh > 0) {
-                  const unsigned r16 = (unsigned)((hsh[i >> 2] >> (16 * (i & 3))) & 0xFFFFu);
-                  d = r16 >= (unsigned)p.gnb_drop_thresh ? d * p.gnb_drop_scale : 0.f;
-                }
-                if (p.gnb_silu) {
-                  const float h = fmaf(xv, kc.x, kc.y);
-                  d *= P == kBF16X3 ? dsilu_ex2_half(h) : dsilu_tanh_half(h);
-                }
-                v[i] = d;
-                q2[i] = d * fmaf(xv, kc.z, kc.w);
-              }
-            } else {
-#pragma unroll
-              for (int i = 0; i < 32; ++i) q2[i] = 0.f;
-            }
-          }
-          if (!GNB && p.res && valid) {
-            if (P == kTF32 || p.res_fp32) {
-              if (full) {
-                add_res_chunk<kTF32>(rbuf, v);
-              } else {
-                const float* rp = reinterpret_cast<const float*>(p.res) + roff + nb;
-                for (int i = 0; i < 32; ++i) if (nb + i < p.N) v[i] += rp[i];
-              }
-            } else {
-              if (full) {
-                add_res_chunk<P>(rbuf, v);
-              } else {
-                const ActElem<P>* rp = reinterpret_cast<const ActElem<P>*>(p.res) + roff + nb;
-                for (int i = 0; i < 32; ++i) if (nb + i < p.N) v[i] += load_split<P>(rp + i, p.res_lo_off);
-              }
-            }
-          }
-          if (ch + kChunkStep < kChunks) prefetch_res(ch + kChunkStep);
-          if (valid) {
-            if (p.out_fp32) {
-              float* op = reinterpret_cast<float*>(p.out) + ooff + nb;
-              if (full) {
-#pragma unroll
-                for (int i = 0; i < 8; ++i) reinterpret_cast<float4*>(op)[i] = make_float4(v[4 * i], v[4 * i + 1], v[4 * i + 2], v[4 * i + 3]);
-              } else {
-                for (int i = 0; i < 32; ++i) if (nb + i < p.N) op[i * p.ocs] = v[i];
-              }
-            } else {
-              ActElem<P>* op = reinterpret_cast<ActElem<P>*>(p.out) + ooff + nb;
-              if (full) {
-                constexpr int E = kVecElems<P>;
-#pragma unroll
-                for (int i = 0; i < 32 / E; ++i) store_vec<P>(op + E * i, p.out_lo_off * (long long)sizeof(ActElem<P>), v + E * i);
-              } else {
-                for (int i = 0; i < 32; ++i) if (nb + i < p.N) store_split<P>(op + i * p.ocs, p.out_lo_off, v[i]);
-              }
-            }
-          }
-          if (GNB ? (want_cols != 0) : (p.stats != nullptr)) {
-            float s[32], ss[32];
-#pragma unroll
-            for (int i = 0; i < 32; ++i) {
-              const float t = valid ? v[i] : 0.f;
-              s[i] = t; ss[i] = GNB ? q2[GNB ? i : 0] : t * t;
-            }
-            colsum_butterfly<16>(s, ss, lane);
-            s_part[(q * 2 + 0) * BLOCK_N + ch * 32 + lane] = s[0];
-            s_part[(q * 2 + 1) * BLOCK_N + ch * 32 + lane] = ss[0];
-          }
-        }
-      }
-      if constexpr (GNB) {
-        if (p.gnb_part && splits == 1) {
-          named_bar_sync(1, kEpiThreads);
-          const int warps_per_seg = rows_per_b >= 128 ? 4 : rows_per_b / 32;
+        stage();
+        if constexpr (Cfg::kStageRounds > 1) {
+#pragma unroll
+          for (int i = 0; i < kRoundRegs; ++i) acc[i] = acc[kRoundRegs + i];
+        }
+
+        const int bkey = p.rowbias ? b0 : 0;
+        if (n0 != staged_n0 || bkey != staged_b0) {
+          staged_n0 = n0; staged_b0 = bkey;
+          bias_buf ^= 1;
+          float* wb = s_stats + 16 * BLOCK_N + bias_buf * 4 * BLOCK_N;
           for (int i = et; i < p.bb * BLOCK_N; i += kEpiThreads) {
             const int sg = i / BLOCK_N, c = i % BLOCK_N;
-            const int n = n0 + c;
-            if (mt_of_tile < tiles_m && n < p.N) {
-              float ts = 0.f, tq = 0.f;
-              for (int w = sg * warps_per_seg; w < (sg + 1) * warps_per_seg; ++w) {
-                ts += s_part[(w * 2 + 0) * BLOCK_N + c];
-                tq += s_part[(w * 2 + 1) * BLOCK_N + c];
-              }
-              float* dst = p.gnb_part + ((static_cast<long long>(mt_of_tile) * p.bb + sg) * p.N + n) * 2;
-              dst[0] = ts; dst[1] = tq;
-            }
-          }
-        }
-      }
-      if (!GNB && p.stats && splits == 1) {
-        named_bar_sync(1, kEpiThreads);
-        const int warps_per_seg = rows_per_b >= 128 ? 4 : rows_per_b / 32;
-        for (int i0 = 0; i0 < p.bb * BLOCK_N; i0 += kEpiThreads) {
-          const int i = i0 + et;
-          const int sg = i / BLOCK_N, c = i % BLOCK_N;
-          const int bgl = b0 + sg, n = n0 + c;
-          if (i < p.bb * BLOCK_N && bgl < p.Bn && n < p.N) {
-            float ts = 0.f, tq = 0.f;
-            for (int w = sg * warps_per_seg; w < (sg + 1) * warps_per_seg; ++w) {
-              ts += s_part[(w * 2 + 0) * BLOCK_N + c];
-              tq += s_part[(w * 2 + 1) * BLOCK_N + c];
-            }
-            long long* dst = p.stats + (static_cast<long long>(bgl) * p.N + n) * kStatWords;
-            stat_add(dst, ts);
-            stat_add(dst + 2, tq);
-          }
+            const int n = n0 + c, bgl = b0 + sg;
+            float bv = 0.f;
+            if (n < p.N) {
+              if (p.bias && !p.bias_on_m) bv += __ldg(p.bias + n);
+              if (p.rowbias && bgl < p.Bn) bv += __ldg(p.rowbias + static_cast<long long>(bgl) * p.rowbias_ld + n);
+            }
+            wb[i] = bv;
+          }
+        }
+        const float* s_bias = s_stats + 16 * BLOCK_N + bias_buf * 4 * BLOCK_N;
+        float* s_part = s_stats + (vit & 1) * 8 * BLOCK_N;
+        uint4 rbuf[8];
+        auto prefetch_res = [&](int ch) {
+          const int nbp = n0 + ch * 32;
+          if (!(p.res && valid && p.ocs == 1 && nbp + 32 <= p.N)) return;
+          if constexpr (GNB) {
+            const bool second = p.res1 && nbp >= p.res_c0;
+            const __nv_bfloat16* base = reinterpret_cast<const __nv_bfloat16*>(second ? p.res1 : p.res);
+            const long long off = second ? xg * p.r1sx + yg * p.r1sy + zg * p.r1sz + bg * p.r1sb + (nbp - p.res_c0) : roff + nbp;
+            const uint4* rp = reinterpret_cast<const uint4*>(base + off);
+#pragma unroll
+            for (int i = 0; i < 4; ++i) rbuf[i] = __ldg(rp + i);
+            if constexpr (P == kBF16X3) {
+              const uint4* rl = reinterpret_cast<const uint4*>(base + off + (second ? p.res1_lo_off : p.res_lo_off));
+#pragma unroll
+              for (int i = 0; i < 4; ++i) rbuf[4 + i] = __ldg(rl + i);
+            }
+            return;
+          }
+          if (P == kTF32 || p.res_fp32) {
+            const uint4* rp = reinterpret_cast<const uint4*>(reinterpret_cast<const float*>(p.res) + roff + nbp);
+#pragma unroll
+            for (int i = 0; i < 8; ++i) rbuf[i] = __ldg(rp + i);
+          } else {
+            const uint4* rp = reinterpret_cast<const uint4*>(reinterpret_cast<const __nv_bfloat16*>(p.res) + roff + nbp);
+#pragma unroll
+            for (int i = 0; i < 4; ++i) rbuf[i] = __ldg(rp + i);
+            if constexpr (P == kBF16X3) {
+              const uint4* rl = reinterpret_cast<const uint4*>(reinterpret_cast<const __nv_bfloat16*>(p.res) + roff + nbp + p.res_lo_off);
+#pragma unroll
+              for (int i = 0; i < 4; ++i) rbuf[4 + i] = __ldg(rl + i);
+            }
+          }
+        };
+        const int ch0 = kChunkStep == 2 ? half : 0;
+        const bool active = kChunkStep == 2 || half == 0;
+        if (active) prefetch_res(ch0);
+
+        constexpr int kRoundChunks = Cfg::kStageCols / 32;
+#pragma unroll 1
+        for (int rnd = 0; rnd < Cfg::kStageRounds; ++rnd) {
+          if (rnd > 0) {
+            named_bar_sync(2, kEpiThreads);
+            stage();
+          }
+          named_bar_sync(2, kEpiThreads);
+
+#pragma unroll 1
+          for (int ch = ch0 + rnd * kRoundChunks; ch < (rnd + 1) * kRoundChunks && active; ch += kChunkStep) {
+            uint32_t rr[32];
+            {
+              const float4* src = reinterpret_cast<const float4*>(s_acc + row * Cfg::kAccPitch + (ch - rnd * kRoundChunks) * 32);
+#pragma unroll
+              for (int i = 0; i < 8; ++i) {
+                const float4 t = src[i];
+                rr[4 * i] = __float_as_uint(t.x); rr[4 * i + 1] = __float_as_uint(t.y);
+                rr[4 * i + 2] = __float_as_uint(t.z); rr[4 * i + 3] = __float_as_uint(t.w);
+              }
+            }
+            const int nb = n0 + ch * 32;
+            if (nb >= p.N) continue;
+            if (splits > 1) {
+              if (valid) {
+                float* pp = p.partial + (long long)(tile % splits) * p.split_stride + (P == kBF16X3 ? (ooff >> 1) : ooff) + nb;
+                if (nb + 32 <= p.N) {
+#pragma unroll
+                  for (int i = 0; i < 8; ++i)
+                    reinterpret_cast<float4*>(pp)[i] = make_float4(__uint_as_float(rr[4 * i]), __uint_as_float(rr[4 * i + 1]),
+                                                                   __uint_as_float(rr[4 * i + 2]), __uint_as_float(rr[4 * i + 3]));
+                } else {
+                  for (int i = 0; i < 32; ++i) if (nb + i < p.N) pp[i] = __uint_as_float(rr[i]);
+                }
+              }
+              continue;
+            }
+            const bool full = (nb + 32 <= p.N) && (p.ocs == 1);
+            float v[32];
+            const float mbias = (p.bias && p.bias_on_m && valid) ? __ldg(p.bias + xg) : 0.f;
+            const float* sb = s_bias + (seg < 4 ? seg : 0) * BLOCK_N + ch * 32;
+#pragma unroll
+            for (int i = 0; i < 32; ++i) v[i] = __uint_as_float(rr[i]) * p.alpha + mbias + sb[i];
+            float q2[GNB ? 32 : 1];
+            if constexpr (GNB) {
+              if (valid) {
+                const float4* cc = p.gnb_c + static_cast<long long>(bg) * p.N + nb;
+                unsigned long long hsh[8];
+                if (p.gnb_drop_thresh > 0) {
+                  const unsigned long long e4 = (unsigned long long)((((static_cast<long long>(bg) * p.Z + zg) * p.Y + yg) * p.X + xg) * p.N + nb) >> 2;
+#pragma unroll
+                  for (int i = 0; i < 8; ++i) hsh[i] = drop_hash64(p.gnb_seed, e4 + i);
+                }
+#pragma unroll
+                for (int i = 0; i < 32; ++i) {
+                  const float4 kc = __ldg(cc + i);
+                  const __nv_bfloat16 xb = reinterpret_cast<const __nv_bfloat16*>(rbuf)[i];
+                  float xv = __bfloat162float(xb);
+                  if constexpr (P == kBF16X3) xv += __bfloat162float(reinterpret_cast<const __nv_bfloat16*>(rbuf + 4)[i]);
+                  float d = v[i];
+                  if (p.gnb_drop_thresh > 0) {
+                    const unsigned r16 = (unsigned)((hsh[i >> 2] >> (16 * (i & 3))) & 0xFFFFu);
+                    d = r16 >= (unsigned)p.gnb_drop_thresh ? d * p.gnb_drop_scale : 0.f;
+                  }
+                  if (p.gnb_silu) {
+                    const float h = fmaf(xv, kc.x, kc.y);
+                    d *= P == kBF16X3 ? dsilu_ex2_half(h) : dsilu_tanh_half(h);
+                  }
+                  v[i] = d;
+                  q2[i] = d * fmaf(xv, kc.z, kc.w);
+                }
+              } else {
+#pragma unroll
+                for (int i = 0; i < 32; ++i) q2[i] = 0.f;
+              }
+            }
+            if (!GNB && p.res && valid) {
+              if (P == kTF32 || p.res_fp32) {
+                if (full) {
+                  add_res_chunk<kTF32>(rbuf, v);
+                } else {
+                  const float* rp = reinterpret_cast<const float*>(p.res) + roff + nb;
+                  for (int i = 0; i < 32; ++i) if (nb + i < p.N) v[i] += rp[i];
+                }
+              } else {
+                if (full) {
+                  add_res_chunk<P>(rbuf, v);
+                } else {
+                  const ActElem<P>* rp = reinterpret_cast<const ActElem<P>*>(p.res) + roff + nb;
+                  for (int i = 0; i < 32; ++i) if (nb + i < p.N) v[i] += load_split<P>(rp + i, p.res_lo_off);
+                }
+              }
+            }
+            if (ch + kChunkStep < kChunks) prefetch_res(ch + kChunkStep);
+            if (valid) {
+              if (p.out_fp32) {
+                float* op = reinterpret_cast<float*>(p.out) + ooff + nb;
+                if (full) {
+#pragma unroll
+                  for (int i = 0; i < 8; ++i) reinterpret_cast<float4*>(op)[i] = make_float4(v[4 * i], v[4 * i + 1], v[4 * i + 2], v[4 * i + 3]);
+                } else {
+                  for (int i = 0; i < 32; ++i) if (nb + i < p.N) op[i * p.ocs] = v[i];
+                }
+              } else {
+                ActElem<P>* op = reinterpret_cast<ActElem<P>*>(p.out) + ooff + nb;
+                if (full) {
+                  constexpr int E = kVecElems<P>;
+#pragma unroll
+                  for (int i = 0; i < 32 / E; ++i) store_vec<P>(op + E * i, p.out_lo_off * (long long)sizeof(ActElem<P>), v + E * i);
+                } else {
+                  for (int i = 0; i < 32; ++i) if (nb + i < p.N) store_split<P>(op + i * p.ocs, p.out_lo_off, v[i]);
+                }
+              }
+            }
+            if (GNB ? (want_cols != 0) : (p.stats != nullptr)) {
+              float s[32], ss[32];
+#pragma unroll
+              for (int i = 0; i < 32; ++i) {
+                const float t = valid ? v[i] : 0.f;
+                s[i] = t; ss[i] = GNB ? q2[GNB ? i : 0] : t * t;
+              }
+              colsum_butterfly<16>(s, ss, lane);
+              s_part[(q * 2 + 0) * BLOCK_N + ch * 32 + lane] = s[0];
+              s_part[(q * 2 + 1) * BLOCK_N + ch * 32 + lane] = ss[0];
+            }
+          }
+        }
+        if constexpr (GNB) {
+          if (p.gnb_part && splits == 1) {
+            named_bar_sync(1, kEpiThreads);
+            const int warps_per_seg = rows_per_b >= 128 ? 4 : rows_per_b / 32;
+            for (int i = et; i < p.bb * BLOCK_N; i += kEpiThreads) {
+              const int sg = i / BLOCK_N, c = i % BLOCK_N;
+              const int n = n0 + c;
+              if (mt_of_tile < tiles_m && n < p.N) {
+                float ts = 0.f, tq = 0.f;
+                for (int w = sg * warps_per_seg; w < (sg + 1) * warps_per_seg; ++w) {
+                  ts += s_part[(w * 2 + 0) * BLOCK_N + c];
+                  tq += s_part[(w * 2 + 1) * BLOCK_N + c];
+                }
+                float* dst = p.gnb_part + ((static_cast<long long>(mt_of_tile) * p.bb + sg) * p.N + n) * 2;
+                dst[0] = ts; dst[1] = tq;
+              }
+            }
+          }
+        }
+      } else {
+        int x0, y0, z0, b0, n0;
+        decode(tile, x0, y0, z0, b0, n0);
+
+        constexpr int kRoundRegs = Cfg::kStageCols / 2;
+        auto stage = [&]() {
+          const int w4 = (warp & 3), srow = wg * 64 + w4 * 16 + (lane >> 2), scol = 2 * (lane & 3);
+#pragma unroll
+          for (int j = 0; j < Cfg::kStageCols / 8; ++j) {
+            *reinterpret_cast<float2*>(s_acc + srow * Cfg::kAccPitch + 8 * j + scol) = make_float2(acc[4 * j], acc[4 * j + 1]);
+            *reinterpret_cast<float2*>(s_acc + (srow + 8) * Cfg::kAccPitch + 8 * j + scol) = make_float2(acc[4 * j + 2], acc[4 * j + 3]);
+          }
+        };
+        named_bar_sync(2, kEpiThreads);
+        stage();
+        if constexpr (Cfg::kStageRounds > 1) {
+#pragma unroll
+          for (int i = 0; i < kRoundRegs; ++i) acc[i] = acc[kRoundRegs + i];
+        }
+
+        const int bkey = p.rowbias ? b0 : 0;
+        if (n0 != staged_n0 || bkey != staged_b0) {
+          staged_n0 = n0; staged_b0 = bkey;
+          bias_buf ^= 1;
+          stage_bias<BLOCK_N>(p, s_stats + 16 * BLOCK_N + bias_buf * 4 * BLOCK_N, n0, b0, et, kEpiThreads);
+        }
+        const float* s_bias = s_stats + 16 * BLOCK_N + bias_buf * 4 * BLOCK_N;
+        float* s_part = s_stats + (vit & 1) * 8 * BLOCK_N;
+        EpiRow<BLOCK_N, P, GNB> er(p, tile, splits, row, x0, y0, z0, b0, n0);
+        const int ch0 = kChunkStep == 2 ? half : 0;
+        const bool active = kChunkStep == 2 || half == 0;
+        if (active) er.prefetch_res(ch0);
+
+        constexpr int kRoundChunks = Cfg::kStageCols / 32;
+#pragma unroll 1
+        for (int rnd = 0; rnd < Cfg::kStageRounds; ++rnd) {
+          if (rnd > 0) {
+            named_bar_sync(2, kEpiThreads);
+            stage();
+          }
+          named_bar_sync(2, kEpiThreads);
+
+#pragma unroll 1
+          for (int ch = ch0 + rnd * kRoundChunks; ch < (rnd + 1) * kRoundChunks && active; ch += kChunkStep) {
+            uint32_t rr[32];
+            {
+              const float4* src = reinterpret_cast<const float4*>(s_acc + row * Cfg::kAccPitch + (ch - rnd * kRoundChunks) * 32);
+#pragma unroll
+              for (int i = 0; i < 8; ++i) {
+                const float4 t = src[i];
+                rr[4 * i] = __float_as_uint(t.x); rr[4 * i + 1] = __float_as_uint(t.y);
+                rr[4 * i + 2] = __float_as_uint(t.z); rr[4 * i + 3] = __float_as_uint(t.w);
+              }
+            }
+            er.chunk(ch, ch + kChunkStep < kChunks ? ch + kChunkStep : -1, rr, s_bias, seg, s_part, q, lane, want_cols);
+          }
+        }
+        if (p.stats && splits == 1) {
+          named_bar_sync(1, kEpiThreads);
+          column_stats<BLOCK_N>(p, s_part, n0, b0, et, kEpiThreads);
         }
       }
     }
diff --git a/meshdiffusion_b200/diffusion/models/ddpm.py b/meshdiffusion_b200/diffusion/models/ddpm.py
--- a/meshdiffusion_b200/diffusion/models/ddpm.py
+++ b/meshdiffusion_b200/diffusion/models/ddpm.py
@@ -507,6 +507,15 @@
             rows.append((a.value, b.value, sm.value))
         return rows
 
+    def gemm_epilogues(self):
+        L = _native.lib()
+        rows = []
+        for i in range(self.engine_info()["gemm_launches"]):
+            h = ctypes.c_int()
+            _native.check(L.mdb_unet_gemm_epilogue(self._handle, i, ctypes.byref(h)))
+            rows.append("handoff" if h.value else "inline")
+        return rows
+
     def gemm_tiles(self):
         L = _native.lib()
         rows = []
```

After: 36.88, median of 6. 1.01x the previous value.
